# valida-xyz/valida

Measured on AMD Instinct MI355X. Metric: proofs/sec, 2^20-row Fibonacci trace, higher is better.
Workload: dtype u32; 1 GPU; C2: Fibonacci 2^20 cpu rows (mem 2^22), 14 chips, one proof per GPU; field=BabyBear / Ext5, mmcs=Keccak-256, fri_blowup=2, log_blowup=1, num_queries=40, pow_bits=8, parallelism=single GPU, proofs_in_flight_per_gpu=3, comm_stuck=False

## Files before the change

### bindings/rust/src/lib.rs

```rust
#![allow(non_camel_case_types, dead_code)]
use core::ffi::{c_char, c_int, c_void};

pub const VGPU_CBOR_CANONICAL_FIELDS: u32 = 1;
pub const VGPU_CBOR_PLAIN_DIGESTS: u32 = 2;
pub const VGPU_CBOR_IN_BARE_IS_MONTGOMERY: u32 = 1;
pub const VGPU_CBOR_SAW_FIELD_STRUCT: u32 = 1;
pub const VGPU_CBOR_SAW_FIELD_BARE: u32 = 2;
pub const VGPU_CBOR_SAW_DIGEST_STRUCT: u32 = 4;
pub const VGPU_CBOR_SAW_DIGEST_PLAIN: u32 = 8;
pub const VGPU_COMM_ID_BYTES: u32 = 128;
pub const VGPU_OK: i32 = 0;
pub const VGPU_ERR_INVALID_ARG: i32 = -1;
pub const VGPU_ERR_OOM: i32 = -2;
pub const VGPU_ERR_HIP: i32 = -3;
pub const VGPU_ERR_UNSUPPORTED: i32 = -4;
pub const VGPU_ERR_INTERNAL: i32 = -5;
pub const VGPU_ERR_FABRIC: i32 = -6;
pub const VGPU_HASH_KECCAK256: i32 = 0;
pub const VGPU_HASH_POSEIDON16: i32 = 1;
pub const VGPU_CPU_STORE32: i32 = 0;
pub const VGPU_CPU_LOAD32: i32 = 1;
pub const VGPU_CPU_JAL: i32 = 2;
pub const VGPU_CPU_JALV: i32 = 3;
pub const VGPU_CPU_BEQ: i32 = 4;
// ... 239 lines not shown
    pub mem_first: u32,
}
#[repr(C)]
#[derive(Clone, Copy)]
pub struct VgpuMemOp {
    pub clk: u32,
    pub addr: u32,
    pub value: u32,
    pub is_write: u32,
}
#[repr(C)]
#[derive(Clone, Copy)]
pub struct VgpuAluOp {
    pub opcode: u32,
    pub a: u32,
    pub b: u32,
    pub c: u32,
}
#[repr(C)]
#[derive(Clone, Copy)]
pub struct VgpuOutOp {
    pub clk: u32,
    pub byte: u32,
}
#[repr(C)]
#[derive(Clone, Copy)]
pub struct VgpuOplogDesc {
    pub struct_size: u64,
    pub cpu: *const VgpuCpuOp,
    pub n_cpu: u64,
    pub mem: *const VgpuMemOp,
    pub n_mem: u64,
    pub alu: [*const VgpuAluOp; 4],
    pub n_alu: [u64; 4],
    pub static_cells: *const u32,
    pub n_static: u64,
    pub rom_len: u32,
    pub alu2: [*const VgpuAluOp; 4],
    pub n_alu2: [u64; 4],
    pub output: *const VgpuOutOp,
    pub n_output: u64,
}

#[link(name = "vgpu")]
extern "C" {
    pub fn vgpu_last_error() -> *const c_char;
    pub fn vgpu_version() -> *const c_char;
    pub fn vgpu_air_new(name: *const c_char, width: u32, preprocessed_width: u32, out: *mut *mut VgpuAir) -> i32;
    pub fn vgpu_air_free(air: *mut VgpuAir);
    pub fn vgpu_air_constant(air: *mut VgpuAir, canonical: u32) -> u32;
    pub fn vgpu_air_variable(air: *mut VgpuAir, is_preprocessed: u32, column: u32, is_next: u32) -> u32;
    pub fn vgpu_air_is_first_row(air: *mut VgpuAir) -> u32;
    pub fn vgpu_air_is_last_row(air: *mut VgpuAir) -> u32;
    pub fn vgpu_air_is_transition(air: *mut VgpuAir) -> u32;
    pub fn vgpu_air_add(air: *mut VgpuAir, a: u32, b: u32) -> u32;
    pub fn vgpu_air_sub(air: *mut VgpuAir, a: u32, b: u32) -> u32;
    pub fn vgpu_air_mul(air: *mut VgpuAir, a: u32, b: u32) -> u32;
    pub fn vgpu_air_neg(air: *mut VgpuAir, a: u32) -> u32;
    pub fn vgpu_air_assert_zero(air: *mut VgpuAir, node: u32);
    pub fn vgpu_air_add_interaction(air: *mut VgpuAir, it: *const VgpuInteraction) -> i32;
    pub fn vgpu_machine_new(out: *mut *mut VgpuMachine) -> i32;
    pub fn vgpu_machine_push_air(m: *mut VgpuMachine, air: *const VgpuAir) -> i32;
    pub fn vgpu_machine_basic(out: *mut *mut VgpuMachine) -> i32;
    pub fn vgpu_machine_basic_via_ffi(out: *mut *mut VgpuMachine) -> i32;
    pub fn vgpu_machine_free(m: *mut VgpuMachine);
    pub fn vgpu_machine_num_chips(m: *const VgpuMachine) -> u32;
    pub fn vgpu_machine_chip_info(m: *const VgpuMachine, chip: u32, out: *mut u32) -> i32;
    pub fn vgpu_machine_interaction_words(m: *const VgpuMachine, chip: u32, out: *mut u32, cap: u64) -> i64;
    pub fn vgpu_machine_eval_constraints(m: *const VgpuMachine, chip: u32, main_local: *const u32, main_next: *const u32, prep_local: *const u32, prep_next: *const u32, is_first: u32, is_last: u32, is_transition: u32, out: *mut u32, cap: u32) -> i32;
    pub fn vgpu_challenger_new(poseidon_rc: *const u32, out: *mut *mut VgpuChallenger) -> i32;
    pub fn vgpu_challenger_free(ch: *mut VgpuChallenger);
    pub fn vgpu_challenger_observe(ch: *mut VgpuChallenger, values: *const u32, n: u64);
    pub fn vgpu_challenger_sample(ch: *mut VgpuChallenger, out: *mut u32, n: u64);
    pub fn vgpu_challenger_sample_bits(ch: *mut VgpuChallenger, bits: u32) -> u64;
    pub fn vgpu_challenger_grind(ch: *mut VgpuChallenger, bits: u32) -> u32;
    pub fn vgpu_poseidon16_permute(poseidon_rc: *const u32, state: *mut u32);
    pub fn vgpu_poseidon16_permute_sparse(poseidon_rc: *const u32, state: *mut u32) -> i32;
    pub fn vgpu_prover_create(cfg: *const VgpuConfig, machine: *const VgpuMachine, out: *mut *mut VgpuProver) -> i32;
    pub fn vgpu_prover_destroy(p: *mut VgpuProver);
    pub fn vgpu_prover_memory(p: *const VgpuProver, live_bytes: *mut u64, peak_bytes: *mut u64);
    pub fn vgpu_prover_trim(p: *mut VgpuProver) -> u64;
    pub fn vgpu_prover_memory_reset_peak(p: *mut VgpuProver);
    pub fn vgpu_prover_set_dense_lane(p: *mut VgpuProver, on: u32, min_nodes: u64);
    pub fn vgpu_prover_lane_stats(p: *const VgpuProver, entered: *mut u64, waited: *mut u64);
    pub fn vgpu_prover_set_profiling(p: *mut VgpuProver, on: u32);
    pub fn vgpu_prover_set_prep_cache(p: *mut VgpuProver, on: u32);
    pub fn vgpu_prover_set_profiling_filter(p: *mut VgpuProver, kernel_name: *const c_char);
    pub fn vgpu_prover_profile(p: *mut VgpuProver, out: *mut c_char, cap: u64) -> i64;
    pub fn vgpu_shader_clock_probe(device: i32, iters: u32, out: *mut u64) -> i32;
    pub fn vgpu_host_alloc(bytes: u64, out: *mut *mut c_void) -> i32;
    pub fn vgpu_host_free(ptr: *mut c_void);
    pub fn vgpu_trace_upload(p: *mut VgpuProver, data: *const u32, height: u64, width: u64, out: *mut *mut VgpuTrace) -> i32;
    pub fn vgpu_trace_free(t: *mut VgpuTrace);
    pub fn vgpu_commit_batches(p: *mut VgpuProver, mats: *const *const VgpuTrace, n_mats: u32, coset_shifts: *const u32, root: *mut u32, out: *mut *mut VgpuPdata) -> i32;
    pub fn vgpu_pdata_lde(p: *mut VgpuProver, pd: *const VgpuPdata, idx: u32, out: *mut u32, cap_words: u64) -> i32;
    pub fn vgpu_pdata_num_matrices(pd: *const VgpuPdata) -> u32;
    pub fn vgpu_pdata_lde_view(pd: *const VgpuPdata, idx: u32, out: *mut VgpuLdeView) -> i32;
    pub fn vgpu_pdata_free(pd: *mut VgpuPdata);
    pub fn vgpu_perm_trace(p: *mut VgpuProver, chip: u32, main: *const VgpuTrace, preprocessed_or_null: *const VgpuTrace, challenges: *const u32, out: *mut u32, cap_words: u64, cumulative_sum: *mut u32) -> i32;
    pub fn vgpu_perm_trace_device(p: *mut VgpuProver, chip: u32, main: *const VgpuTrace, preprocessed_or_null: *const VgpuTrace, challenges: *const u32, out: *mut *mut VgpuTrace, cumulative_sum: *mut u32) -> i32;
    pub fn vgpu_quotient(p: *mut VgpuProver, chip: u32, prep_pd: *const VgpuPdata, prep_idx: u32, main_pd: *const VgpuPdata, main_idx: u32, perm_pd: *const VgpuPdata, perm_idx: u32, perm_challenges: *const u32, alpha: *const u32, cumulative_sum: *const u32, out: *mut *mut VgpuTrace) -> i32;
    pub fn vgpu_open_multi_batches(p: *mut VgpuProver, rounds: *const *const VgpuPdata, n_rounds: u32, n_points: *const u32, points: *const u32, ch: *mut VgpuChallenger, out: *mut *mut VgpuOpening) -> i32;
    pub fn vgpu_opening_values_len(o: *const VgpuOpening) -> u64;
    pub fn vgpu_opening_values(o: *const VgpuOpening) -> *const u32;
    pub fn vgpu_opening_proof_len(o: *const VgpuOpening) -> u64;
    pub fn vgpu_opening_proof(o: *const VgpuOpening) -> *const u32;
    pub fn vgpu_opening_free(o: *mut VgpuOpening);
    pub fn vgpu_verify_multi_batches(cfg: *const VgpuConfig, commits: *const u32, n_rounds: u32, n_mats: *const u32, heights: *const u64, widths: *const u32, n_points: *const u32, points: *const u32, values: *const u32, n_value_words: u64, proof: *const u32, n_proof_words: u64, ch: *mut VgpuChallenger) -> i32;
    pub fn vgpu_verify(cfg: *const VgpuConfig, machine: *const VgpuMachine, preprocessed_commit: *const u32, proof_words: *const u32, n_words: u64) -> i32;
    pub fn vgpu_verifier_create(cfg: *const VgpuConfig, machine: *const VgpuMachine, out: *mut *mut VgpuVerifier) -> i32;
    pub fn vgpu_verifier_destroy(v: *mut VgpuVerifier);
    pub fn vgpu_verifier_set_chunk_words(v: *mut VgpuVerifier, chunk_words: u64) -> i32;
    pub fn vgpu_verify_batch(v: *mut VgpuVerifier, proofs: *const *const u32, n_words: *const u64, preprocessed_commits: *const u32, n_proofs: u32, status: *mut i32) -> i32;
    pub fn vgpu_verifier_message(v: *const VgpuVerifier, i: u32, out: *mut c_char, cap: u64) -> i64;
    pub fn vgpu_verifier_timing(v: *const VgpuVerifier, host_ms: *mut f64, device_ms: *mut f64);
    pub fn vgpu_host_commit_root(cfg: *const VgpuConfig, mats: *const *const u32, heights: *const u64, widths: *const u64, n_mats: u32, coset_shifts: *const u32, root: *mut u32) -> i32;
    pub fn vgpu_fri_fold(p: *mut VgpuProver, f: *const u32, n: u64, beta: *const u32, out: *mut u32) -> i32;
    pub fn vgpu_field_probe(p: *mut VgpuProver, op: u32, operands: *const u32, operand_words: u64, n_items: u64, results: *mut u32, result_words: u64) -> i32;
    pub fn vgpu_prover_set_pool_poison(p: *mut VgpuProver, mode: u32, word: u32) -> i32;
    pub fn vgpu_prover_pool_poison_stats(p: *const VgpuProver, out: *mut u64);
    pub fn vgpu_prover_pool_peek(p: *mut VgpuProver, bytes: u64, out: *mut u32, n_words: u64) -> i32;
    pub fn vgpu_verifier_set_poison(v: *mut VgpuVerifier, on: u32, word: u32) -> i32;
    pub fn vgpu_prove(p: *mut VgpuProver, main: *const *const VgpuTrace, n_main: u32, prep_chips: *const u32, prep: *const *const VgpuTrace, n_prep: u32, debug_flags: u32, out: *mut *mut VgpuProof) -> i32;
    pub fn vgpu_prove_async(p: *mut VgpuProver, main: *const *const VgpuTrace, n_main: u32, prep_chips: *const u32, prep: *const *const VgpuTrace, n_prep: u32, out: *mut *mut VgpuTicket) -> i32;
    pub fn vgpu_ticket_wait(t: *mut VgpuTicket, out: *mut *mut VgpuProof) -> i32;
    pub fn vgpu_proof_cbor(proof_words: *const u32, n_words: u64, flags: u32, out: *mut u8, cap_bytes: u64) -> i64;
    pub fn vgpu_proof_from_cbor(bytes: *const u8, n_bytes: u64, out: *mut u32, cap_words: u64) -> i64;
    pub fn vgpu_proof_from_cbor_ex(bytes: *const u8, n_bytes: u64, flags: u32, out: *mut u32, cap_words: u64, forms_seen: *mut u32) -> i64;
    pub fn vgpu_proof_len(pr: *const VgpuProof) -> u64;
    pub fn vgpu_proof_words(pr: *const VgpuProof) -> *const u32;
    pub fn vgpu_proof_phase_ms(pr: *const VgpuProof, out: *mut f64);
    pub fn vgpu_proof_transcript(pr: *const VgpuProof, out: *mut u32);
    pub fn vgpu_proof_debug_perm_trace(pr: *const VgpuProof, chip: u32, out: *mut u32, cap_words: u64) -> i64;
    pub fn vgpu_proof_debug_quotient(pr: *const VgpuProof, chip: u32, out: *mut u32, cap_words: u64) -> i64;
    pub fn vgpu_proof_free(pr: *mut VgpuProof);
    pub fn vgpu_bus_audit(p: *mut VgpuProver, main: *const *const VgpuTrace, n_main: u32, prep_chips: *const u32, prep: *const *const VgpuTrace, n_prep: u32, opts: *const VgpuBusAuditOpts, out: *mut *mut VgpuBusReport) -> i32;
    pub fn vgpu_bus_audit_host(machine: *const VgpuMachine, main: *const *const u32, heights: *const u64, widths: *const u64, n_main: u32, prep_chips: *const u32, prep: *const *const u32, prep_heights: *const u64, prep_widths: *const u64, n_prep: u32, opts: *const VgpuBusAuditOpts, out: *mut *mut VgpuBusReport) -> i32;
    pub fn vgpu_bus_report_len(r: *const VgpuBusReport) -> u64;
    pub fn vgpu_bus_report_words(r: *const VgpuBusReport) -> *const u32;
    pub fn vgpu_bus_report_timing(r: *const VgpuBusReport, out: *mut f64);
    pub fn vgpu_bus_report_free(r: *mut VgpuBusReport);
    pub fn vgpu_constraint_audit(p: *mut VgpuProver, main: *const *const VgpuTrace, n_main: u32, prep_chips: *const u32, prep: *const *const VgpuTrace, n_prep: u32, opts: *const VgpuConstraintAuditOpts, out: *mut *mut VgpuConstraintReport) -> i32;
    pub fn vgpu_constraint_audit_host(machine: *const VgpuMachine, main: *const *const u32, heights: *const u64, widths: *const u64, n_main: u32, prep_chips: *const u32, prep: *const *const u32, prep_heights: *const u64, prep_widths: *const u64, n_prep: u32, opts: *const VgpuConstraintAuditOpts, out: *mut *mut VgpuConstraintReport) -> i32;
    pub fn vgpu_constraint_report_len(r: *const VgpuConstraintReport) -> u64;
    pub fn vgpu_constraint_report_words(r: *const VgpuConstraintReport) -> *const u32;
    pub fn vgpu_constraint_report_timing(r: *const VgpuConstraintReport, out: *mut f64);
    pub fn vgpu_constraint_report_free(r: *mut VgpuConstraintReport);
    pub fn vgpu_mutation_audit(p: *mut VgpuProver, main: *const *const VgpuTrace, n_main: u32, prep_chips: *const u32, prep: *const *const VgpuTrace, n_prep: u32, opts: *const VgpuMutationAuditOpts, out: *mut *mut VgpuMutationReport) -> i32;
    pub fn vgpu_mutation_audit_host(machine: *const VgpuMachine, main: *const *const u32, heights: *const u64, widths: *const u64, n_main: u32, prep_chips: *const u32, prep: *const *const u32, prep_heights: *const u64, prep_widths: *const u64, n_prep: u32, opts: *const VgpuMutationAuditOpts, out: *mut *mut VgpuMutationReport) -> i32;
    pub fn vgpu_mutation_report_len(r: *const VgpuMutationReport) -> u64;
    pub fn vgpu_mutation_report_words(r: *const VgpuMutationReport) -> *const u32;
    pub fn vgpu_mutation_report_timing(r: *const VgpuMutationReport, out: *mut f64);
    pub fn vgpu_mutation_report_free(r: *mut VgpuMutationReport);
    pub fn vgpu_pair_audit(p: *mut VgpuProver, main: *const *const VgpuTrace, n_main: u32, prep_chips: *const u32, prep: *const *const VgpuTrace, n_prep: u32, opts: *const VgpuPairAuditOpts, out: *mut *mut VgpuPairReport) -> i32;
    pub fn vgpu_pair_audit_host(machine: *const VgpuMachine, main: *const *const u32, heights: *const u64, widths: *const u64, n_main: u32, prep_chips: *const u32, prep: *const *const u32, prep_heights: *const u64, prep_widths: *const u64, n_prep: u32, opts: *const VgpuPairAuditOpts, out: *mut *mut VgpuPairReport) -> i32;
    pub fn vgpu_pair_report_len(r: *const VgpuPairReport) -> u64;
    pub fn vgpu_pair_report_words(r: *const VgpuPairReport) -> *const u32;
    pub fn vgpu_pair_report_timing(r: *const VgpuPairReport, out: *mut f64);
    pub fn vgpu_pair_report_free(r: *mut VgpuPairReport);
    pub fn vgpu_rank_audit(p: *mut VgpuProver, main: *const *const VgpuTrace, n_main: u32, prep_chips: *const u32, prep: *const *const VgpuTrace, n_prep: u32, opts: *const VgpuRankAuditOpts, out: *mut *mut VgpuRankReport) -> i32;
    pub fn vgpu_rank_audit_host(machine: *const VgpuMachine, main: *const *const u32, heights: *const u64, widths: *const u64, n_main: u32, prep_chips: *const u32, prep: *const *const u32, prep_heights: *const u64, prep_widths: *const u64, n_prep: u32, opts: *const VgpuRankAuditOpts, out: *mut *mut VgpuRankReport) -> i32;
    pub fn vgpu_rank_report_len(r: *const VgpuRankReport) -> u64;
    pub fn vgpu_rank_report_words(r: *const VgpuRankReport) -> *const u32;
    pub fn vgpu_rank_report_timing(r: *const VgpuRankReport, out: *mut f64);
    pub fn vgpu_rank_report_free(r: *mut VgpuRankReport);
    pub fn vgpu_field_audit(p: *mut VgpuProver, main: *const *const VgpuTrace, n_main: u32, prep_chips: *const u32, prep: *const *const VgpuTrace, n_prep: u32, opts: *const VgpuRankAuditOpts, out: *mut *mut VgpuFieldReport) -> i32;
    pub fn vgpu_field_audit_host(machine: *const VgpuMachine, main: *const *const u32, heights: *const u64, widths: *const u64, n_main: u32, prep_chips: *const u32, prep: *const *const u32, prep_heights: *const u64, prep_widths: *const u64, n_prep: u32, opts: *const VgpuRankAuditOpts, out: *mut *mut VgpuFieldReport) -> i32;
    pub fn vgpu_field_report_len(r: *const VgpuFieldReport) -> u64;
    pub fn vgpu_field_report_words(r: *const VgpuFieldReport) -> *const u32;
    pub fn vgpu_field_report_timing(r: *const VgpuFieldReport, out: *mut f64);
    pub fn vgpu_field_report_free(r: *mut VgpuFieldReport);
    pub fn vgpu_link_audit(p: *mut VgpuProver, main: *const *const VgpuTrace, n_main: u32, prep_chips: *const u32, prep: *const *const VgpuTrace, n_prep: u32, opts: *const VgpuLinkAuditOpts, out: *mut *mut VgpuLinkReport) -> i32;
    pub fn vgpu_link_audit_host(machine: *const VgpuMachine, main: *const *const u32, heights: *const u64, widths: *const u64, n_main: u32, prep_chips: *const u32, prep: *const *const u32, prep_heights: *const u64, prep_widths: *const u64, n_prep: u32, opts: *const VgpuLinkAuditOpts, out: *mut *mut VgpuLinkReport) -> i32;
    pub fn vgpu_link_report_len(r: *const VgpuLinkReport) -> u64;
    pub fn vgpu_link_report_words(r: *const VgpuLinkReport) -> *const u32;
    pub fn vgpu_link_report_timing(r: *const VgpuLinkReport, out: *mut f64);
    pub fn vgpu_link_report_free(r: *mut VgpuLinkReport);
// ... 82 lines not shown
```

### include/vgpu.h

```cpp
#ifndef VGPU_H
#define VGPU_H
#include <stdint.h>
#ifdef __cplusplus
extern "C" {
#endif

enum {
    VGPU_OK = 0,
    VGPU_ERR_INVALID_ARG = -1,
    VGPU_ERR_OOM = -2,
    VGPU_ERR_HIP = -3,
    VGPU_ERR_UNSUPPORTED = -4,
    VGPU_ERR_INTERNAL = -5,
    VGPU_ERR_FABRIC = -6
};
enum {
    VGPU_HASH_KECCAK256 = 0,
    VGPU_HASH_POSEIDON16 = 1
};

const char* vgpu_last_error(void);
const char* vgpu_version(void);

typedef struct vgpu_config {
    int32_t device;
    uint32_t log_blowup;
    uint32_t num_queries;
    uint32_t pow_bits;
    uint32_t hash_kind;
    uint32_t observe_final_poly;
    uint32_t poseidon_rc[480];
    uint32_t interpret_air;
} vgpu_config_t;

typedef struct vgpu_air vgpu_air_t;
typedef struct vgpu_vcol_term { uint32_t is_preprocessed; uint32_t column; uint32_t weight; } vgpu_vcol_term_t;
typedef struct vgpu_vcol { const vgpu_vcol_term_t* terms; uint32_t n_terms; uint32_t constant; } vgpu_vcol_t;
typedef struct vgpu_interaction {
    const vgpu_vcol_t* fields; uint32_t n_fields;
    vgpu_vcol_t count;
    uint32_t is_global;
    uint32_t bus_index;
    uint32_t is_send;
} vgpu_interaction_t;

int32_t vgpu_air_new(const char* name, uint32_t width, uint32_t preprocessed_width, vgpu_air_t** out);
void vgpu_air_free(vgpu_air_t* air);
uint32_t vgpu_air_constant(vgpu_air_t* air, uint32_t canonical);
uint32_t vgpu_air_variable(vgpu_air_t* air, uint32_t is_preprocessed, uint32_t column, uint32_t is_next);
uint32_t vgpu_air_is_first_row(vgpu_air_t* air);
uint32_t vgpu_air_is_last_row(vgpu_air_t* air);
uint32_t vgpu_air_is_transition(vgpu_air_t* air);
uint32_t vgpu_air_add(vgpu_air_t* air, uint32_t a, uint32_t b);
uint32_t vgpu_air_sub(vgpu_air_t* air, uint32_t a, uint32_t b);
uint32_t vgpu_air_mul(vgpu_air_t* air, uint32_t a, uint32_t b);
uint32_t vgpu_air_neg(vgpu_air_t* air, uint32_t a);
void vgpu_air_assert_zero(vgpu_air_t* air, uint32_t node);
int32_t vgpu_air_add_interaction(vgpu_air_t* air, const vgpu_interaction_t* it);

typedef struct vgpu_machine vgpu_machine_t;
int32_t vgpu_machine_new(vgpu_machine_t** out);
int32_t vgpu_machine_push_air(vgpu_machine_t* m, const vgpu_air_t* air);
int32_t vgpu_machine_basic(vgpu_machine_t** out);
int32_t vgpu_machine_basic_via_ffi(vgpu_machine_t** out);
void vgpu_machine_free(vgpu_machine_t* m);
uint32_t vgpu_machine_num_chips(const vgpu_machine_t* m);
int32_t vgpu_machine_chip_info(const vgpu_machine_t* m, uint32_t chip, uint32_t out[8]);
int64_t vgpu_machine_interaction_words(const vgpu_machine_t* m, uint32_t chip, uint32_t* out, uint64_t cap);
int32_t vgpu_machine_eval_constraints(const vgpu_machine_t* m, uint32_t chip, const uint32_t* main_local, const uint32_t* main_next,
                                      const uint32_t* prep_local, const uint32_t* prep_next, uint32_t is_first, uint32_t is_last,
                                      uint32_t is_transition, uint32_t* out, uint32_t cap);

typedef struct vgpu_challenger vgpu_challenger_t;
int32_t vgpu_challenger_new(const uint32_t poseidon_rc[480], vgpu_challenger_t** out);
void vgpu_challenger_free(vgpu_challenger_t* ch);
void vgpu_challenger_observe(vgpu_challenger_t* ch, const uint32_t* values, uint64_t n);
void vgpu_challenger_sample(vgpu_challenger_t* ch, uint32_t* out, uint64_t n);
uint64_t vgpu_challenger_sample_bits(vgpu_challenger_t* ch, uint32_t bits);
uint32_t vgpu_challenger_grind(vgpu_challenger_t* ch, uint32_t bits);
void vgpu_poseidon16_permute(const uint32_t poseidon_rc[480], uint32_t state[16]);
int32_t vgpu_poseidon16_permute_sparse(const uint32_t poseidon_rc[480], uint32_t state[16]);

typedef struct vgpu_prover vgpu_prover_t;
typedef struct vgpu_trace vgpu_trace_t;
typedef struct vgpu_pdata vgpu_pdata_t;
typedef struct vgpu_proof vgpu_proof_t;

int32_t vgpu_prover_create(const vgpu_config_t* cfg, const vgpu_machine_t* machine, vgpu_prover_t** out);
void vgpu_prover_destroy(vgpu_prover_t* p);
void vgpu_prover_memory(const vgpu_prover_t* p, uint64_t* live_bytes, uint64_t* peak_bytes);
uint64_t vgpu_prover_trim(vgpu_prover_t* p);
void vgpu_prover_memory_reset_peak(vgpu_prover_t* p);
void vgpu_prover_set_dense_lane(vgpu_prover_t* p, uint32_t on, uint64_t min_nodes);
void vgpu_prover_lane_stats(const vgpu_prover_t* p, uint64_t* entered, uint64_t* waited);

void vgpu_prover_set_profiling(vgpu_prover_t* p, uint32_t on);
void vgpu_prover_set_prep_cache(vgpu_prover_t* p, uint32_t on);
void vgpu_prover_set_profiling_filter(vgpu_prover_t* p, const char* kernel_name);
int64_t vgpu_prover_profile(vgpu_prover_t* p, char* out, uint64_t cap);
int32_t vgpu_shader_clock_probe(int32_t device, uint32_t iters, uint64_t out[2]);

int32_t vgpu_host_alloc(uint64_t bytes, void** out);
void vgpu_host_free(void* ptr);

int32_t vgpu_trace_upload(vgpu_prover_t* p, const uint32_t* data, uint64_t height, uint64_t width, vgpu_trace_t** out);
void vgpu_trace_free(vgpu_trace_t* t);

int32_t vgpu_commit_batches(vgpu_prover_t* p, const vgpu_trace_t* const* mats, uint32_t n_mats, const uint32_t* coset_shifts,
                            uint32_t root[8], vgpu_pdata_t** out);
int32_t vgpu_pdata_lde(vgpu_prover_t* p, const vgpu_pdata_t* pd, uint32_t idx, uint32_t* out, uint64_t cap_words);
typedef struct vgpu_lde_view {
    const uint32_t* data;
    uint64_t height, width, stride;
    uint32_t log_blowup;
} vgpu_lde_view_t;
uint32_t vgpu_pdata_num_matrices(const vgpu_pdata_t* pd);
int32_t vgpu_pdata_lde_view(const vgpu_pdata_t* pd, uint32_t idx, vgpu_lde_view_t* out);
void vgpu_pdata_free(vgpu_pdata_t* pd);

int32_t vgpu_perm_trace(vgpu_prover_t* p, uint32_t chip, const vgpu_trace_t* main, const vgpu_trace_t* preprocessed_or_null,
                        const uint32_t challenges[15], uint32_t* out, uint64_t cap_words, uint32_t cumulative_sum[5]);

int32_t vgpu_perm_trace_device(vgpu_prover_t* p, uint32_t chip, const vgpu_trace_t* main, const vgpu_trace_t* preprocessed_or_null,
                               const uint32_t challenges[15], vgpu_trace_t** out, uint32_t cumulative_sum[5]);

int32_t vgpu_quotient(vgpu_prover_t* p, uint32_t chip, const vgpu_pdata_t* prep_pd, uint32_t prep_idx, const vgpu_pdata_t* main_pd, uint32_t main_idx,
                      const vgpu_pdata_t* perm_pd, uint32_t perm_idx, const uint32_t perm_challenges[15], const uint32_t alpha[5],
                      const uint32_t cumulative_sum[5], vgpu_trace_t** out);

typedef struct vgpu_opening vgpu_opening_t;
int32_t vgpu_open_multi_batches(vgpu_prover_t* p, const vgpu_pdata_t* const* rounds, uint32_t n_rounds, const uint32_t* n_points,
                                const uint32_t* points, vgpu_challenger_t* ch, vgpu_opening_t** out);
uint64_t vgpu_opening_values_len(const vgpu_opening_t* o);
const uint32_t* vgpu_opening_values(const vgpu_opening_t* o);
uint64_t vgpu_opening_proof_len(const vgpu_opening_t* o);
const uint32_t* vgpu_opening_proof(const vgpu_opening_t* o);
void vgpu_opening_free(vgpu_opening_t* o);

int32_t vgpu_verify_multi_batches(const vgpu_config_t* cfg, const uint32_t* commits, uint32_t n_rounds, const uint32_t* n_mats, const uint64_t* heights,
                                  const uint32_t* widths, const uint32_t* n_points, const uint32_t* points, const uint32_t* values, uint64_t n_value_words,
                                  const uint32_t* proof, uint64_t n_proof_words, vgpu_challenger_t* ch);

int32_t vgpu_verify(const vgpu_config_t* cfg, const vgpu_machine_t* machine, const uint32_t* preprocessed_commit, const uint32_t* proof_words,
                    uint64_t n_words);
typedef struct vgpu_verifier vgpu_verifier_t;
int32_t vgpu_verifier_create(const vgpu_config_t* cfg, const vgpu_machine_t* machine, vgpu_verifier_t** out);
void vgpu_verifier_destroy(vgpu_verifier_t* v);
int32_t vgpu_verifier_set_chunk_words(vgpu_verifier_t* v, uint64_t chunk_words);
int32_t vgpu_verify_batch(vgpu_verifier_t* v, const uint32_t* const* proofs, const uint64_t* n_words, const uint32_t* preprocessed_commits,
                          uint32_t n_proofs, int32_t* status);
int64_t vgpu_verifier_message(const vgpu_verifier_t* v, uint32_t i, char* out, uint64_t cap);
void vgpu_verifier_timing(const vgpu_verifier_t* v, double* host_ms, double* device_ms);
int32_t vgpu_host_commit_root(const vgpu_config_t* cfg, const uint32_t* const* mats, const uint64_t* heights, const uint64_t* widths, uint32_t n_mats,
                              const uint32_t* coset_shifts, uint32_t root[8]);

int32_t vgpu_fri_fold(vgpu_prover_t* p, const uint32_t* f, uint64_t n, const uint32_t beta[5], uint32_t* out);

int32_t vgpu_field_probe(vgpu_prover_t* p, uint32_t op, const uint32_t* operands, uint64_t operand_words, uint64_t n_items, uint32_t* results, uint64_t result_words);

int32_t vgpu_prover_set_pool_poison(vgpu_prover_t* p, uint32_t mode, uint32_t word);
void vgpu_prover_pool_poison_stats(const vgpu_prover_t* p, uint64_t out[4]);
int32_t vgpu_prover_pool_peek(vgpu_prover_t* p, uint64_t bytes, uint32_t* out, uint64_t n_words);
int32_t vgpu_verifier_set_poison(vgpu_verifier_t* v, uint32_t on, uint32_t word);

int32_t vgpu_prove(vgpu_prover_t* p, const vgpu_trace_t* const* main, uint32_t n_main, const uint32_t* prep_chips,
                   const vgpu_trace_t* const* prep, uint32_t n_prep, uint32_t debug_flags, vgpu_proof_t** out);
typedef struct vgpu_ticket vgpu_ticket_t;
int32_t vgpu_prove_async(vgpu_prover_t* p, const vgpu_trace_t* const* main, uint32_t n_main, const uint32_t* prep_chips,
                         const vgpu_trace_t* const* prep, uint32_t n_prep, vgpu_ticket_t** out);
int32_t vgpu_ticket_wait(vgpu_ticket_t* t, vgpu_proof_t** out);
#define VGPU_CBOR_CANONICAL_FIELDS 1u
#define VGPU_CBOR_PLAIN_DIGESTS 2u
int64_t vgpu_proof_cbor(const uint32_t* proof_words, uint64_t n_words, uint32_t flags, uint8_t* out, uint64_t cap_bytes);
int64_t vgpu_proof_from_cbor(const uint8_t* bytes, uint64_t n_bytes, uint32_t* out, uint64_t cap_words);
#define VGPU_CBOR_IN_BARE_IS_MONTGOMERY 1u
#define VGPU_CBOR_SAW_FIELD_STRUCT 1u
#define VGPU_CBOR_SAW_FIELD_BARE 2u
#define VGPU_CBOR_SAW_DIGEST_STRUCT 4u
#define VGPU_CBOR_SAW_DIGEST_PLAIN 8u
int64_t vgpu_proof_from_cbor_ex(const uint8_t* bytes, uint64_t n_bytes, uint32_t flags, uint32_t* out, uint64_t cap_words, uint32_t* forms_seen);
uint64_t vgpu_proof_len(const vgpu_proof_t* pr);
const uint32_t* vgpu_proof_words(const vgpu_proof_t* pr);
void vgpu_proof_phase_ms(const vgpu_proof_t* pr, double out[11]);
void vgpu_proof_transcript(const vgpu_proof_t* pr, uint32_t out[33]);
int64_t vgpu_proof_debug_perm_trace(const vgpu_proof_t* pr, uint32_t chip, uint32_t* out, uint64_t cap_words);
int64_t vgpu_proof_debug_quotient(const vgpu_proof_t* pr, uint32_t chip, uint32_t* out, uint64_t cap_words);
void vgpu_proof_free(vgpu_proof_t* pr);

typedef struct vgpu_bus_audit_opts { uint64_t max_tuples; uint32_t max_records_per_tuple; uint32_t hash_bits; } vgpu_bus_audit_opts_t;
typedef struct vgpu_bus_report vgpu_bus_report_t;
int32_t vgpu_bus_audit(vgpu_prover_t* p, const vgpu_trace_t* const* main, uint32_t n_main, const uint32_t* prep_chips, const vgpu_trace_t* const* prep,
                       uint32_t n_prep, const vgpu_bus_audit_opts_t* opts, vgpu_bus_report_t** out);
// ... 339 lines not shown
```

### valida_amd/__init__.py

```python
import ctypes
import os

import numpy as np

P = 2013265921
NUM_CHIPS = 14
CHIP_NAMES = ["cpu", "program", "mem", "add", "sub", "mul", "div", "shift", "lt", "com", "bitwise", "output", "range", "static_data"]

_HERE = os.path.dirname(os.path.abspath(__file__))
_LIB_PATH = os.environ.get("VGPU_LIB_PATH") or os.path.join(_HERE, "libvgpu.so")

c_u32p = ctypes.POINTER(ctypes.c_uint32)
c_u64p = ctypes.POINTER(ctypes.c_uint64)


HASH_KECCAK256, HASH_POSEIDON16 = 0, 1


class VgpuError(RuntimeError):
    def __init__(self, code, msg):
        super().__init__("vgpu error %d: %s" % (code, msg))
        self.code = code


# ... 1973 lines not shown
        return cls(cls._image(first.deltas, False, len(listed), chips, listed))


def _coverage_opts(deltas, max_cells, max_workgroups):
    if int(max_cells) < 1:
        raise VgpuError(-1, "coverage_audit: max_cells must be at least 1")
    ds = [int(d) for d in ((1, P - 1) if deltas is None else deltas)]
    if not 1 <= len(ds) <= 4:
        raise VgpuError(-1, "coverage_audit: 1 to 4 deltas (got %d)" % len(ds))
    if any(d < 0 or d > 0xFFFFFFFF for d in ds):
        raise VgpuError(-1, "coverage_audit: a delta must be a canonical value in 1..p-1")
    if not 0 <= int(max_workgroups) <= 0xFFFFFFFF:
        raise VgpuError(-1, "coverage_audit: max_workgroups is a 32-bit count (0: the default)")
    return CoverageAuditOpts(int(max_cells), len(ds), (ctypes.c_uint32 * 4)(*ds), int(max_workgroups), (ctypes.c_uint32 * 2)(0, 0))


def coverage_audit_host(machine, main_matrices, preprocessed, deltas=None, max_cells=8192):
    opts = _coverage_opts(deltas, max_cells, 0)
    return _audit_host("coverage", machine, main_matrices, preprocessed, opts)


_AUDIT_REPORTS = dict(bus=BusReport, constraint=ConstraintReport, mutation=MutationReport, pair=PairReport, rank=RankReport, step=StepReport, invariant=InvariantReport, transition=TransitionReport, product=ProductReport, domain=DomainReport, memory=MemoryReport, program=ProgramReport, field=FieldReport,
                      link=LinkReport, coverage=CoverageReport)


def _report_of(name):
    return lambda h: _audit_report(name, _AUDIT_REPORTS[name], h)


_rank_report, _step_report, _field_report, _link_report = _report_of("rank"), _report_of("step"), _report_of("field"), _report_of("link")

def _pool_poison_from_env(environ):
    text = environ.get("VGPU_POOL_POISON", "").strip()
    if not text:
        return None
    hexa = text[:2] in ("0x", "0X")
    digits = text[2:] if hexa else text
    if not digits or any(ch not in ("0123456789abcdefABCDEF" if hexa else "0123456789") for ch in digits):
        raise ValueError("VGPU_POOL_POISON must be a 32-bit word in decimal or 0x hex, not %r" % text)
    word = int(digits, 16 if hexa else 10)
    if word > 0xFFFFFFFF:
        raise ValueError("VGPU_POOL_POISON must be a 32-bit word (at most 0xFFFFFFFF), not %r" % text)
    return word


class Ticket:

    def __init__(self, handle, keep):
        self._h, self._keep = handle, keep

    def wait(self):
        h = ctypes.c_void_p()
        t, self._h = self._h, None
        _check(lib().vgpu_ticket_wait(t, ctypes.byref(h)))
        self._keep = None
        return Proof(h)

    def __del__(self):
        if getattr(self, "_h", None):
            try:
                self.wait()
            except Exception:
                pass


class Prover:

    def __init__(self, machine, rc, device=0, log_blowup=1, num_queries=40, pow_bits=8, observe_final_poly=False, interpret_air=False, hash_kind=HASH_KECCAK256):
        cfg = VgpuConfig()
        cfg.device, cfg.log_blowup, cfg.num_queries, cfg.pow_bits = device, log_blowup, num_queries, pow_bits
        cfg.hash_kind, cfg.observe_final_poly, cfg.interpret_air = int(hash_kind), int(observe_final_poly), int(interpret_air)
        rc = np.ascontiguousarray(rc, dtype=np.uint32)
        assert rc.size == 480
        ctypes.memmove(cfg.poseidon_rc, rc.ctypes.data, 480 * 4)
        self.machine, self.rc, self.log_blowup, self.num_queries, self.pow_bits = machine, rc, log_blowup, num_queries, pow_bits
        self._h = ctypes.c_void_p()
        lane_off, lane_min = os.environ.get("VGPU_DENSE_LANE", "1") == "0", os.environ.get("VGPU_DENSE_LANE_MIN_NODES", "").strip()
        if lane_min and not lane_min.isdigit():
            raise ValueError("VGPU_DENSE_LANE_MIN_NODES must be a number of leaf rows, not %r" % lane_min)
        poison = _pool_poison_from_env(os.environ)
        _check(lib().vgpu_prover_create(ctypes.byref(cfg), machine._h, ctypes.byref(self._h)))
        if lane_off or int(lane_min or 0) > 0:
            self.set_dense_lane(not lane_off, int(lane_min or 0))
        if poison is not None:
            self.set_pool_poison(poison)

    def set_dense_lane(self, on, min_nodes=0):
        lib().vgpu_prover_set_dense_lane(self._h, ctypes.c_uint32(1 if on else 0), ctypes.c_uint64(int(min_nodes)))

    def upload(self, matrix):
        m = np.ascontiguousarray(matrix, dtype=np.uint32)
        assert m.ndim == 2
        h = ctypes.c_void_p()
        _check(lib().vgpu_trace_upload(self._h, m.ctypes.data_as(c_u32p), ctypes.c_uint64(m.shape[0]), ctypes.c_uint64(m.shape[1]), ctypes.byref(h)))
        return DeviceTrace(self, h, m.shape)

    def upload_oplog(self, desc):
        h = ctypes.c_void_p()
        _check(lib().vgpu_oplog_upload(self._h, ctypes.byref(desc), ctypes.byref(h)))
        nbytes = 48 * desc.n_cpu + 16 * desc.n_mem + 16 * sum(desc.n_alu) + 8 * desc.n_static
        log = DeviceOplog(self, h, int(nbytes))
        log._desc = desc
        return log

    def generate_trace(self, log, chip):
        h = ctypes.c_void_p()
        _check(lib().vgpu_generate_trace(self._h, log._h, ctypes.c_uint32(chip), ctypes.byref(h)))
        hh, ww = ctypes.c_uint64(), ctypes.c_uint64()
        lib().vgpu_trace_shape(h, ctypes.byref(hh), ctypes.byref(ww))
        return DeviceTrace(self, h, (int(hh.value), int(ww.value)))

    def commit_batches(self, traces, coset_shifts=None):
        arr = (ctypes.c_void_p * len(traces))(*[t._h for t in traces])
        root = np.zeros(8, dtype=np.uint32)
        sh = None
        if coset_shifts is not None:
            shv, sh = _u32(coset_shifts)
        h = ctypes.c_void_p()
        _check(lib().vgpu_commit_batches(self._h, arr, ctypes.c_uint32(len(traces)), sh, root.ctypes.data_as(c_u32p), ctypes.byref(h)))
        return ProverData(self, h, root, [t.shape for t in traces])

    def generate_permutation_trace(self, chip, main, challenges, preprocessed=None):
        info = self.machine.chip_info(chip)
        n = main.shape[0]
        out = np.zeros((n, 5 * (info["interactions"] + 1)), dtype=np.uint32)
        ch, chp = _u32(challenges)
        cs = np.zeros(5, dtype=np.uint32)
        _check(lib().vgpu_perm_trace(self._h, ctypes.c_uint32(chip), main._h, preprocessed._h if preprocessed is not None else None, chp,
                                     out.ctypes.data_as(c_u32p), ctypes.c_uint64(out.size), cs.ctypes.data_as(c_u32p)))
        return out, cs

    def permutation_trace_device(self, chip, main, challenges, preprocessed=None):
        ch, chp = _u32(challenges)
        cs = np.zeros(5, dtype=np.uint32)
        h = ctypes.c_void_p()
        _check(lib().vgpu_perm_trace_device(self._h, ctypes.c_uint32(chip), main._h, preprocessed._h if preprocessed is not None else None, chp, ctypes.byref(h),
                                            cs.ctypes.data_as(c_u32p)))
        hh, ww = ctypes.c_uint64(), ctypes.c_uint64()
        lib().vgpu_trace_shape(h, ctypes.byref(hh), ctypes.byref(ww))
        return DeviceTrace(self, h, (int(hh.value), int(ww.value))), cs

    def quotient(self, chip, main_pd, main_idx, perm_pd, perm_idx, perm_challenges, alpha, cumulative_sum, prep_pd=None, prep_idx=0):
        a, ap = _u32(perm_challenges)
        b, bp = _u32(alpha)
        c, cp = _u32(cumulative_sum)
        h = ctypes.c_void_p()
        _check(lib().vgpu_quotient(self._h, ctypes.c_uint32(chip), prep_pd._h if prep_pd is not None else None, ctypes.c_uint32(prep_idx), main_pd._h,
                                   ctypes.c_uint32(main_idx), perm_pd._h, ctypes.c_uint32(perm_idx), ap, bp, cp, ctypes.byref(h)))
        hh, ww = ctypes.c_uint64(), ctypes.c_uint64()
        lib().vgpu_trace_shape(h, ctypes.byref(hh), ctypes.byref(ww))
        return DeviceTrace(self, h, (int(hh.value), int(ww.value)))

    def open_multi_batches(self, rounds, points, challenger):
        arr = (ctypes.c_void_p * len(rounds))(*[r._h for r in rounds])
        n_points = np.array([len(pts) for rnd in points for pts in rnd], dtype=np.uint32)
        flat = np.array([w for rnd in points for pts in rnd for z in pts for w in z], dtype=np.uint32)
        h = ctypes.c_void_p()
        _check(lib().vgpu_open_multi_batches(self._h, arr, ctypes.c_uint32(len(rounds)), n_points.ctypes.data_as(c_u32p), flat.ctypes.data_as(c_u32p), challenger._h,
                                             ctypes.byref(h)))
        L = lib()
        for f in (L.vgpu_opening_values_len, L.vgpu_opening_proof_len):
            f.restype = ctypes.c_uint64
        for f in (L.vgpu_opening_values, L.vgpu_opening_proof):
            f.restype = c_u32p
        try:
            nv, npf = int(L.vgpu_opening_values_len(h)), int(L.vgpu_opening_proof_len(h))
            vals = np.ctypeslib.as_array(L.vgpu_opening_values(h), shape=(nv,)).copy() if nv else np.zeros(0, np.uint32)
            proof = np.ctypeslib.as_array(L.vgpu_opening_proof(h), shape=(npf,)).copy()
        finally:
            L.vgpu_opening_free(h)
        out, pos = [], 0
        for r, rnd in enumerate(points):
            out.append([])
            for i, pts in enumerate(rnd):
                w = rounds[r]._shapes[i][1]
                out[r].append([])
                for _ in pts:
                    out[r][i].append(vals[pos:pos + 5 * w].reshape(w, 5))
                    pos += 5 * w
        assert pos == vals.size
        return out, proof

    def fri_fold(self, f, beta):
        f = np.ascontiguousarray(f, dtype=np.uint32)
        n = f.shape[0]
        b, bp = _u32(beta)
        out = np.zeros((n // 2, 5), dtype=np.uint32)
        _check(lib().vgpu_fri_fold(self._h, f.ctypes.data_as(c_u32p), ctypes.c_uint64(n), bp, out.ctypes.data_as(c_u32p)))
        return out

    def prove(self, main, preprocessed, debug=False, check=False):
        arr = (ctypes.c_void_p * len(main))(*[t._h for t in main])
        chips = (ctypes.c_uint32 * max(1, len(preprocessed)))(*[c for c, _ in preprocessed])
        parr = (ctypes.c_void_p * max(1, len(preprocessed)))(*[t._h for _, t in preprocessed])
        h = ctypes.c_void_p()
        _check(lib().vgpu_prove(self._h, arr, ctypes.c_uint32(len(main)), chips, parr, ctypes.c_uint32(len(preprocessed)),
                                ctypes.c_uint32((1 if debug else 0) | (2 if check else 0)), ctypes.byref(h)))
        return Proof(h)

    def _audit(self, name, main, preprocessed, opts):
        arr = (ctypes.c_void_p * max(1, len(main)))(*[t._h for t in main])
        chips = (ctypes.c_uint32 * max(1, len(preprocessed)))(*[c for c, _ in preprocessed])
        parr = (ctypes.c_void_p * max(1, len(preprocessed)))(*[t._h for _, t in preprocessed])
# ... 126 lines not shown
```

### valida_amd/csrc/capi.cpp

```cpp
#include "../../include/vgpu.h"
#include <algorithm>
#include <cstring>
#include <future>
#include <map>
#include <mutex>
#include <memory>
#include <string>
#include "host/cbor.hpp"
#include "host/comm.hpp"
#include "host/sharded.hpp"
#include "host/sharded_prover.hpp"
#include "host/verifier.hpp"
#include "host/machine_verifier.hpp"
#include "host/verify_batch.hpp"
#include "host/poseidon_opt.hpp"
#include "host/prover.hpp"
#include "workload/basic_vm.hpp"
#include "workload/executable.hpp"

using namespace vhost;

static thread_local std::string g_err;
static int32_t fail(int32_t code, const std::string& msg) { g_err = msg; return code; }
#define VG_TRY(...)                                                         \
// ... 231 lines not shown
    };
    const auto& its = m->desc.airs[chip].interactions;
    w.push_back((uint32_t)its.size());
    for (auto& it : its) {
        w.push_back(it.is_send() ? 1u : 0u); w.push_back(it.is_local() ? 0u : 1u); w.push_back((uint32_t)it.bus_index); w.push_back((uint32_t)it.fields.size());
        vcol(it.count);
        for (auto& f : it.fields) vcol(f);
    }
    if (out && cap >= w.size()) memcpy(out, w.data(), w.size() * 4);
    return (int64_t)w.size();
}
int32_t vgpu_machine_eval_constraints(const vgpu_machine_t* m, uint32_t chip, const uint32_t* main_local, const uint32_t* main_next,
                                      const uint32_t* prep_local, const uint32_t* prep_next, uint32_t is_first, uint32_t is_last,
                                      uint32_t is_transition, uint32_t* out, uint32_t cap) {
    try {
        if (!m || chip >= m->desc.airs.size()) throw std::invalid_argument("bad chip index");
        const AirDesc& a = m->desc.airs[chip];
        std::vector<Fp> ml(a.width), mn(a.width), pl(a.prep_width), pn(a.prep_width);
        for (uint32_t i = 0; i < a.width; i++) { ml[i] = Fp::from_canonical(main_local[i]); mn[i] = Fp::from_canonical(main_next[i]); }
        for (uint32_t i = 0; i < a.prep_width; i++) { pl[i] = Fp::from_canonical(prep_local[i]); pn[i] = Fp::from_canonical(prep_next[i]); }
        vair::HostEval ev{ml.data(), mn.data(), pl.data(), pn.data(), Fp::from_canonical(is_first), Fp::from_canonical(is_last), Fp::from_canonical(is_transition)};
        auto vals = ev.run(a.program);
        if (vals.size() > cap) throw std::invalid_argument("output buffer too small");
        for (size_t i = 0; i < vals.size(); i++) out[i] = vals[i].canonical();
        return (int32_t)vals.size();
    } catch (const std::exception& e) { return fail(VGPU_ERR_INVALID_ARG, e.what()); }
}

int32_t vgpu_challenger_new(const uint32_t rc[480], vgpu_challenger_t** out) {
    VG_TRY({
        if (!rc || !out) throw std::invalid_argument("null argument");
        auto* c = new vgpu_challenger();
        c->perm.reset(new Poseidon16(rc));
        c->ch.reset(new Challenger(c->perm.get()));
        *out = c;
    })
}
void vgpu_challenger_free(vgpu_challenger_t* ch) { delete ch; }
void vgpu_challenger_observe(vgpu_challenger_t* ch, const uint32_t* v, uint64_t n) { for (uint64_t i = 0; i < n; i++) ch->ch->observe_canonical(v[i]); }
void vgpu_challenger_sample(vgpu_challenger_t* ch, uint32_t* out, uint64_t n) { for (uint64_t i = 0; i < n; i++) out[i] = ch->ch->sample().canonical(); }
uint64_t vgpu_challenger_sample_bits(vgpu_challenger_t* ch, uint32_t bits) { return ch->ch->sample_bits(bits); }
uint32_t vgpu_challenger_grind(vgpu_challenger_t* ch, uint32_t bits) { return ch->ch->grind(bits); }
void vgpu_poseidon16_permute(const uint32_t rc[480], uint32_t state[16]) {
    Poseidon16 p(rc);
    Fp st[16];
    for (int i = 0; i < 16; i++) st[i] = Fp::from_canonical(state[i]);
    p.permute(st);
    for (int i = 0; i < 16; i++) state[i] = st[i].canonical();
}

int32_t vgpu_poseidon16_permute_sparse(const uint32_t rc[480], uint32_t state[16]) {
    Poseidon16 p(rc);
    PoseidonOptTables t(p);
    if (!t.valid) return VGPU_ERR_UNSUPPORTED;
    Fp st[16];
    for (int i = 0; i < 16; i++) st[i] = Fp::from_canonical(state[i]);
    t.permute(p, st);
    for (int i = 0; i < 16; i++) state[i] = st[i].canonical();
    return VGPU_OK;
}

int32_t vgpu_prover_create(const vgpu_config_t* cfg, const vgpu_machine_t* machine, vgpu_prover_t** out) {
    VG_TRY({
        if (!cfg || !machine || !out) throw std::invalid_argument("null argument");
        if (cfg->hash_kind != VGPU_HASH_KECCAK256 && cfg->hash_kind != VGPU_HASH_POSEIDON16) { g_err = "hash_kind must be VGPU_HASH_KECCAK256 or VGPU_HASH_POSEIDON16"; return VGPU_ERR_UNSUPPORTED; }
        if (cfg->log_blowup < 1 || cfg->log_blowup > 4) throw std::invalid_argument("log_blowup must be in 1..4");
        int count = 0;
        if (hipGetDeviceCount(&count) != hipSuccess || count <= cfg->device) throw std::runtime_error("hip: no usable device (the product path has no CPU fallback)");
        FriParams fp;
        fp.log_blowup = cfg->log_blowup; fp.num_queries = cfg->num_queries; fp.pow_bits = cfg->pow_bits; fp.observe_final_poly = cfg->observe_final_poly != 0;
        fp.interpret_air = cfg->interpret_air != 0;
        fp.hash_kind = (int)cfg->hash_kind;
        auto* p = new vgpu_prover();
        p->p.reset(new Prover(cfg->device, machine->desc, cfg->poseidon_rc, fp));
        *out = p;
    })
}
void vgpu_prover_destroy(vgpu_prover_t* p) { delete p; }
void vgpu_prover_memory(const vgpu_prover_t* p, uint64_t* live, uint64_t* peak) {
    auto& c = const_cast<vgpu_prover_t*>(p)->p->ctx();
    if (live) *live = c.live;
    if (peak) *peak = c.peak_live;
}
void vgpu_prover_set_dense_lane(vgpu_prover_t* p, uint32_t on, uint64_t min_nodes) {
    if (!p) return;
    DeviceCtx& c = p->p->ctx();
    std::lock_guard<std::mutex> lk(c.prove_mu);
    c.lane_on = on != 0;
    if (min_nodes) c.lane_min_nodes = min_nodes;
}
void vgpu_prover_lane_stats(const vgpu_prover_t* p, uint64_t* entered, uint64_t* waited) {
    if (!p) return;
    auto& c = const_cast<vgpu_prover_t*>(p)->p->ctx();
    if (entered) *entered = c.lane_entered.load();
    if (waited) *waited = c.lane_waited.load();
}
void vgpu_prover_memory_reset_peak(vgpu_prover_t* p) {
    if (!p) return;
    DeviceCtx& c = p->p->ctx();
    std::lock_guard<std::mutex> lk(c.pool_mu);
    c.peak_live = c.live;
}
uint64_t vgpu_prover_trim(vgpu_prover_t* p) {
    if (!p) return 0;
    DeviceCtx& c = p->p->ctx();
    (void)hipSetDevice(c.device);
    return (uint64_t)c.trim();
}
void vgpu_prover_set_profiling(vgpu_prover_t* p, uint32_t on) {
    auto& c = p->p->ctx();
    c.profiler.reset();
    c.profiler.enabled = on != 0;
}
int32_t vgpu_shader_clock_probe(int32_t device, uint32_t iters, uint64_t out[2]) {
    VG_TRY({
        if (!out || !iters) throw std::invalid_argument("shader_clock_probe: null output or zero iterations");
        struct Probe { hipStream_t st = nullptr; uint64_t* buf = nullptr; };
        static std::mutex mu;
        static std::map<int, Probe> probes;
        std::lock_guard<std::mutex> lk(mu);
        VG_HIP_CHECK(hipSetDevice(device));
        Probe& pr = probes[device];
        if (!pr.st) {
            VG_HIP_CHECK(hipStreamCreateWithFlags(&pr.st, hipStreamNonBlocking));
            VG_HIP_CHECK(hipHostMalloc((void**)&pr.buf, 64));
        }
        pr.buf[0] = pr.buf[1] = 0;
        vk::launch_clock_probe(pr.st, pr.buf, iters);
        VG_HIP_CHECK(hipStreamSynchronize(pr.st));
        if (!pr.buf[1]) throw std::runtime_error("hip: the clock probe wrote nothing");
        out[0] = pr.buf[0]; out[1] = pr.buf[1];
    })
}
void vgpu_prover_set_prep_cache(vgpu_prover_t* p, uint32_t on) { if (p) p->p->set_prep_cache(on != 0); }
void vgpu_prover_set_profiling_filter(vgpu_prover_t* p, const char* kernel_name) { p->p->ctx().profiler.only = kernel_name ? kernel_name : ""; }
int64_t vgpu_prover_profile(vgpu_prover_t* p, char* out, uint64_t cap) {
    std::string s;
    {
        DeviceCtx& c = p->p->ctx();
        (void)hipSetDevice(c.device);
        (void)hipDeviceSynchronize();
        c.profiler.collect();
    }
    for (auto& kv : p->p->ctx().profiler.stats) {
        char line[256];
        snprintf(line, sizeof line, "%s %llu %.6f %.0f %.0f\n", kv.first.c_str(), (unsigned long long)kv.second.launches, kv.second.ms, kv.second.bytes,
                 kv.second.valu_ops);
        s += line;
    }
    if (out && cap > s.size()) memcpy(out, s.c_str(), s.size() + 1);
    return (int64_t)s.size() + 1;
}
int32_t vgpu_host_alloc(uint64_t bytes, void** out) {
    VG_TRY({
        if (!out || !bytes) throw std::invalid_argument("vgpu_host_alloc: null output or zero size");
        void* ptr = nullptr;
        hipError_t e = hipHostMalloc(&ptr, bytes, hipHostMallocPortable);
        if (e == hipErrorOutOfMemory) throw std::bad_alloc();
        if (e != hipSuccess) throw std::runtime_error(std::string("hipHostMalloc: ") + hipGetErrorString(e));
        *out = ptr;
    })
}
void vgpu_host_free(void* ptr) { if (ptr) (void)hipHostFree(ptr); }
int32_t vgpu_trace_upload(vgpu_prover_t* p, const uint32_t* data, uint64_t height, uint64_t width, vgpu_trace_t** out) {
    VG_TRY({
        if (!p || !data || !out || !height || !width) throw std::invalid_argument("bad trace");
// ... 36 lines not shown
                if (!good) throw std::invalid_argument(std::string("oplog: ") + chip + " log entry " + std::to_string(i) + " has an opcode that is not an operation of that chip");
                if (k == 2 && h.alu2[k][i].c >= 32) throw std::invalid_argument("oplog: shift log entry " + std::to_string(i) + ": shift amount >= 32");
            }
        };
        check(0, {OP_MUL32, OP_MULHS32, OP_MULHU32}, "mul");
        check(1, {OP_DIV32, OP_SDIV32}, "div");
        check(2, {OP_SHL32, OP_SHR32, OP_SRA32}, "shift");
        check(3, {OP_NE32, OP_EQ32}, "com");
    }
    for (uint64_t i = 1; i < h.n_static; i++)
        if (log->static_cells[2 * i] <= log->static_cells[2 * i - 2]) throw std::invalid_argument("oplog: static cells must be in ascending address order");
    if (!h.n_cpu || !log->cpu) throw std::invalid_argument("oplog: empty cpu log");
    if ((h.n_mem && !log->mem) || (h.n_static && !log->static_cells)) throw std::invalid_argument("oplog: null log with a nonzero length");
    for (int k = 0; k < 4; k++) if (h.n_alu[k] && !h.alu[k]) throw std::invalid_argument("oplog: null ALU log with a nonzero length");
    for (uint64_t i = 0; i < h.n_cpu; i++) {
        const vgpu_cpu_op_t& o = log->cpu[i];
        if (o.mem_first > h.n_mem || (i && o.mem_first < log->cpu[i - 1].mem_first) || o.kind > VGPU_CPU_READ_ADVICE)
            throw std::invalid_argument("oplog: cpu record " + std::to_string(i) + " is malformed");
        if (h.rom_len && o.pc >= h.rom_len) throw std::invalid_argument("oplog: cpu record " + std::to_string(i) + ": pc beyond the ROM length");
        if (o.kind == VGPU_CPU_BUS || o.kind == VGPU_CPU_BUS_LEFT_IMM) {
            using namespace vchips;
            const uint32_t op = o.opcode;
            const bool known = (op >= OP_ADD32 && op <= OP_SLE32) || op == OP_WRITE;
            if (!known) throw std::invalid_argument("oplog: cpu record " + std::to_string(i) + ": opcode " + std::to_string(op) + " is no bus operation of the BasicMachine's chips");
        }
    }
    for (uint64_t i = 1; i < h.n_mem; i++)
        if (log->mem[i].clk < log->mem[i - 1].clk) throw std::invalid_argument("oplog: memory log entry " + std::to_string(i) + " is out of clock order");
    return h;
}
int32_t vgpu_oplog_validate(const vgpu_oplog_desc_t* log) {
    VG_TRY({
        if (!log) throw std::invalid_argument("null argument");
        checked_oplog(log);
    })
}
int32_t vgpu_oplog_upload(vgpu_prover_t* p, const vgpu_oplog_desc_t* log, vgpu_oplog_t** out) {
    VG_TRY({
        if (!p || !log || !out) throw std::invalid_argument("null argument");
        const HostOplog h = checked_oplog(log);
        p->p->ctx().activate();
        std::unique_ptr<vgpu_oplog> l(new vgpu_oplog());
        l->owner = p->p;
        l->log = p->p->upload_oplog(h);
        *out = l.release();
    })
}
void vgpu_oplog_free(vgpu_oplog_t* log) { delete log; }
int32_t vgpu_generate_trace(vgpu_prover_t* p, const vgpu_oplog_t* log, uint32_t chip, vgpu_trace_t** out) {
    VG_TRY({
        if (!p || !log || !out) throw std::invalid_argument("null argument");
        p->p->ctx().activate();
        std::unique_ptr<vgpu_trace> t(new vgpu_trace());
        t->owner = p->p;
        t->t = p->p->generate_trace(*log->log, (int)chip);
        *out = t.release();
    })
}

static DMat ingest(DeviceCtx& c, const DeviceTrace& t) {
    if (t.height & (t.height - 1)) throw std::invalid_argument("matrix height must be a power of two");
    DMat m(&c, t.height, t.width);
    if (!t.nat.empty()) VG_HIP_CHECK(hipMemcpyAsync(m.data, t.nat.data, t.height * t.width * 4, hipMemcpyDeviceToDevice, c.stream));
    else vk::launch_ingest(c.stream, t.raw.data, m.view(), false);
    return m;
}

int32_t vgpu_commit_batches(vgpu_prover_t* p, const vgpu_trace_t* const* mats, uint32_t n_mats, const uint32_t* coset_shifts, uint32_t root[8],
                            vgpu_pdata_t** out) {
    VG_TRY({
        if (!p || !mats || !n_mats || !root || !out) throw std::invalid_argument("null argument");
        DeviceCtx& c = p->p->ctx();
        c.activate();
        std::vector<DMat> nat;
        for (uint32_t i = 0; i < n_mats; i++) { if (!mats[i] || mats[i]->owner != p->p) throw std::invalid_argument("null trace or trace of another prover"); nat.push_back(ingest(c, *mats[i]->t)); }
        std::vector<CommitInput> in;
        for (uint32_t i = 0; i < n_mats; i++) in.push_back({&nat[i], mats[i]->t->nat_rows_bitrev, mats[i]->t->nat_rows_bitrev});
        std::vector<Fp> shifts;
        if (coset_shifts) for (uint32_t i = 0; i < n_mats; i++) shifts.push_back(Fp::from_canonical(coset_shifts[i]));
        std::unique_ptr<vgpu_pdata> pd(new vgpu_pdata());
        pd->owner = p->p;
        pd->pd = commit_batches(&c, in, coset_shifts ? &shifts : nullptr, p->p->fri());
        memcpy(root, pd->pd->tree.root, 32);
        *out = pd.release();
    })
}
int32_t vgpu_pdata_lde(vgpu_prover_t* p, const vgpu_pdata_t* pd, uint32_t idx, uint32_t* out, uint64_t cap_words) {
    VG_TRY({
        if (!p || !pd || idx >= pd->pd->ldes.size() || !out) throw std::invalid_argument("bad argument");
        DeviceCtx& c = p->p->ctx();
        c.activate();
        const DMat& l = pd->pd->ldes[idx];
        if (cap_words < l.height * l.width) throw std::invalid_argument("output buffer too small");
        DBuf tmp(&c, (size_t)(l.height * l.width));
        vk::launch_export_rows(c.stream, l.view(), 0, l.height, tmp.data);
        c.download(out, tmp.data, l.height * l.width * 4);
    })
}
uint32_t vgpu_pdata_num_matrices(const vgpu_pdata_t* pd) { return pd ? (uint32_t)pd->pd->ldes.size() : 0; }
int32_t vgpu_pdata_lde_view(const vgpu_pdata_t* pd, uint32_t idx, vgpu_lde_view_t* out) {
    VG_TRY({
        if (!pd || !out || idx >= pd->pd->ldes.size()) throw std::invalid_argument("bad argument");
        const DMat& l = pd->pd->ldes[idx];
        out->data = l.data; out->height = l.height; out->width = l.width; out->stride = l.height;
        out->log_blowup = pd->owner->fri().log_blowup;
    })
}
void vgpu_pdata_free(vgpu_pdata_t* pd) { delete pd; }

static Ext5 ext_of(const uint32_t* w) { Ext5 e; for (int k = 0; k < 5; k++) e.c[k] = Fp::from_canonical(w[k]); return e; }

int32_t vgpu_perm_trace_device(vgpu_prover_t* p, uint32_t chip, const vgpu_trace_t* main, const vgpu_trace_t* prep, const uint32_t challenges[15],
                               vgpu_trace_t** out, uint32_t cumulative_sum[5]) {
    VG_TRY({
        if (!p || !main || !challenges || !out) throw std::invalid_argument("null argument");
        const MachineDesc& md = p->p->machine();
        if (chip >= md.airs.size()) throw std::invalid_argument("bad chip index");
        if (main->t->width != md.airs[chip].width) throw std::invalid_argument("trace width mismatch");
        DeviceCtx& c = p->p->ctx();
        c.activate();
        DMat m = ingest(c, *main->t);
        DMat pm;
        if (prep) pm = ingest(c, *prep->t);
        Ext5 rnd[3] = {ext_of(challenges), ext_of(challenges + 5), ext_of(challenges + 10)};
        Ext5 cs;
        std::unique_ptr<vgpu_trace> t(new vgpu_trace());
        t->owner = p->p;
        t->t = std::make_shared<DeviceTrace>();
        t->t->nat = p->p->permutation_trace((int)chip, m, prep ? &pm : nullptr, rnd, &cs);
        t->t->height = t->t->nat.height; t->t->width = t->t->nat.width;
        if (cumulative_sum) for (int k = 0; k < 5; k++) cumulative_sum[k] = cs.c[k].canonical();
        *out = t.release();
    })
}

int32_t vgpu_quotient(vgpu_prover_t* p, uint32_t chip, const vgpu_pdata_t* prep_pd, uint32_t prep_idx, const vgpu_pdata_t* main_pd, uint32_t main_idx,
                      const vgpu_pdata_t* perm_pd, uint32_t perm_idx, const uint32_t perm_challenges[15], const uint32_t alpha[5],
                      const uint32_t cumulative_sum[5], vgpu_trace_t** out) {
    VG_TRY({
        if (!p || !main_pd || !perm_pd || !perm_challenges || !alpha || !cumulative_sum || !out) throw std::invalid_argument("null argument");
        if (chip >= p->p->machine().airs.size()) throw std::invalid_argument("bad chip index");
        if (main_pd->owner != p->p || perm_pd->owner != p->p || (prep_pd && prep_pd->owner != p->p)) throw std::invalid_argument("prover data of another prover context");
        if (main_idx >= main_pd->pd->ldes.size() || perm_idx >= perm_pd->pd->ldes.size() || (prep_pd && prep_idx >= prep_pd->pd->ldes.size()))
            throw std::invalid_argument("bad matrix index");
        p->p->ctx().activate();
        Ext5 rnd[3] = {ext_of(perm_challenges), ext_of(perm_challenges + 5), ext_of(perm_challenges + 10)};
        std::unique_ptr<vgpu_trace> t(new vgpu_trace());
        t->owner = p->p;
        t->t = std::make_shared<DeviceTrace>();
        t->t->nat = p->p->quotient_chunks((int)chip, main_pd->pd->ldes[main_idx], perm_pd->pd->ldes[perm_idx], prep_pd ? &prep_pd->pd->ldes[prep_idx] : nullptr, rnd,
                                          ext_of(alpha), ext_of(cumulative_sum));
        t->t->nat_rows_bitrev = true;
        t->t->height = t->t->nat.height; t->t->width = t->t->nat.width;
        *out = t.release();
    })
}

int32_t vgpu_open_multi_batches(vgpu_prover_t* p, const vgpu_pdata_t* const* rounds, uint32_t n_rounds, const uint32_t* n_points, const uint32_t* points,
                                vgpu_challenger_t* ch, vgpu_opening_t** out) {
    VG_TRY({
        if (!p || !rounds || !n_rounds || !n_points || !points || !ch || !out) throw std::invalid_argument("null argument");
        std::vector<OpenRound> rs(n_rounds);
        size_t k = 0, w = 0;
        for (uint32_t r = 0; r < n_rounds; r++) {
            if (!rounds[r] || rounds[r]->owner != p->p) throw std::invalid_argument("null prover data or prover data of another prover context");
            rs[r].pd = rounds[r]->pd.get();
// ... 1193 lines not shown
```

### valida_amd/csrc/host/pcs.hpp

```cpp
#pragma once
#include <algorithm>
#include <functional>
#include <memory>
#include "fri_params.hpp"
#include "runtime.hpp"

namespace vhost {


struct ColMat {
    uint64_t height = 0;
    std::vector<const uint32_t*> cols;
};

struct DeviceTree {
    static constexpr uint64_t TOP_FIRST_LEN = 256;
    DeviceCtx* ctx = nullptr;
    std::vector<DBuf> layers;
    std::vector<uint64_t> layer_len;
    unsigned log_max_height = 0;
    uint32_t root[8] = {0};
    static constexpr uint64_t DROP_MIN_LEAVES = 1ull << 16;
    bool drop_bottom = false;
    unsigned dropped = 0;
// ... 84 lines not shown
            vk::launch_poseidon_levels(st, tab, c->poseidon_sparse, pgrp);
            pgrp.levels = 0;
        };
        auto add_level = [&](vk::KeccakTopArgs& g, uint64_t len, const Group* inj) {
            if (g.levels == 0) { g.prev = layers[layers.size() - 2].data; g.first_len = len; }
            g.out[g.levels] = layers.back().data;
            g.cols[g.levels] = inj ? pd + inj->first : nullptr;
            g.n_elems[g.levels] = inj ? (int)inj->count : 0;
            g.levels++;
        };
        auto flush_mid = [&] {
            if (!mid.levels) return;
            mid.block_len = vk::KECCAK_LEVELS_BLOCK_LEN;
            if (leaves_in_mid) {
                if (mid.prev != layers[0].data) throw std::logic_error("mmcs: leaf prologue without a launch over the leaf layer");
                mid.leaf_base = single_view->data; mid.leaf_stride = single_view->stride; mid.leaf_elems = (int)single_view->width; mid.leaf_rows = maxh;
            }
            vk::launch_keccak_levels(st, mid);
            mid.levels = 0;
        };
        for (uint64_t len = maxh / 2; len >= 1; len /= 2) {
            layers.emplace_back(c, (size_t)len * 8);
            layer_len.push_back(len);
            const Group* inj = (gi < groups.size() && groups[gi].height == len) ? &groups[gi] : nullptr;
            if (inj && before_injection_) { (*before_injection_)(); before_injection_ = nullptr; }
            if (pos ? vk::poseidon_levels_take(len) : (len <= TOP_FIRST_LEN || vk::keccak_levels_fused(len))) lane_guard.leave();
            if (pos) {
                if (!vk::poseidon_levels_take(len)) vk::launch_poseidon_compress(st, tab, c->poseidon_sparse, layers[layers.size() - 2].data, inj ? pd + inj->first : nullptr, inj ? (int)inj->count : 0, len, layers.back().data);
                else {
                    if (pgrp.levels && vk::poseidon_levels_group(len) != pgroup) flush_pos(false);
                    pgroup = vk::poseidon_levels_group(len);
                    add_level(pgrp, len, inj);
                }
            } else if (len > TOP_FIRST_LEN) {
                if (vk::keccak_levels_fused(len)) add_level(mid, len, inj);
                else vk::launch_keccak_compress(st, layers[layers.size() - 2].data, inj ? pd + inj->first : nullptr, inj ? (int)inj->count : 0, len,
                                                layers.back().data);
            } else {
                flush_mid();
                add_level(top, len, inj);
            }
            if (inj) gi++;
            if (len == 1) break;
        }
        lane_guard.leave();
        flush_mid();
        if (leaves_in_mid && layers.size() < 2) throw std::logic_error("mmcs: leaf prologue on a tree without parents");
        if (leaves_in_top) {
            if (!top.levels || top.prev != layers[0].data) throw std::logic_error("mmcs: leaf prologue without a top launch over the leaf layer");
            top.leaf_base = single_view->data; top.leaf_stride = single_view->stride; top.leaf_elems = (int)single_view->width; top.leaf_rows = maxh;
        }
        flush_pos(true);
        if (challenger_ && !pos) {
            if (!top.levels) throw std::logic_error("mmcs: the challenger epilogue needs a tree with at least one parent layer");
            top.ch_pos = challenger_->pos; top.ch_state = challenger_->state; top.ch_beta5 = challenger_->beta5; top.ch_commit8 = challenger_->commit8;
        }
        if (top.levels) vk::launch_keccak_top(st, top);
        if (gi != groups.size()) throw std::runtime_error("mmcs: matrix heights must be powers of two >= 1 and <= max height");
        c->check_launch("mmcs build");
        dropped = 0;
        if (drop_bottom && st == c->stream && !c->in_section && maxh >= DROP_MIN_LEAVES && layers.size() >= 4) {
            leaf_elems = (int)groups[0].count;
            if (single) { leaf_ptr = single_view->data; leaf_stride = single_view->stride; }
            else { leaf_ptr = pd + groups[0].first; leaf_stride = 0; }
            layers[0] = DBuf();
            dropped = 1;
            if (!(groups.size() > 1 && groups[1].height == maxh / 2)) { layers[1] = DBuf(); dropped = 2; }
        }
        if (fetch_root) c->download_small(root, layers.back().data, 32);
        if (!fetch_root || dropped) ptr_table_ = std::move(ptr_buf);
    }

};

struct ProverData {
    std::vector<DMat> ldes;
    DeviceTree tree;
};

struct CommitInput {
    DMat* mat;
    bool rows_bitrev;
    bool consume;
};

inline DMat coset_lde(DeviceCtx* c, hipStream_t st, const CommitInput& in, unsigned log_blowup, Fp lde_shift) {
    const uint64_t n = in.mat->height, b = 1ull << log_blowup;
    if (n == 0 || (n & (n - 1))) throw std::invalid_argument("commit: matrix heights must be powers of two");
    if (vg::log2_strict_u64(n) + log_blowup > 27)
        throw std::invalid_argument("commit: LDE height 2^" + std::to_string(vg::log2_strict_u64(n) + log_blowup) + " exceeds the field's two-adicity (2^27)");
    const unsigned k = vg::log2_strict_u64(n);
    static const bool fused = [] { const char* e = getenv("VGPU_LDE_FUSED"); return !(e && e[0] == '0'); }();
    if (!in.rows_bitrev && fused) {
        DMat lde(c, n * b, in.mat->width);
        const vk::LdeTables lt = c->lde_tables((int)k, (int)log_blowup, lde_shift);
        DMat s1, s2;
        if (k > 12) { s1 = DMat(c, n, in.mat->width); s2 = DMat(c, n * b, in.mat->width); }
        vk::launch_lde_natural(st, in.mat->view(), lde.view(), (int)log_blowup, c->tables, lt, s1.empty() ? vk::DMatView{nullptr, 0, 0, 0} : s1.view(),
                               s2.empty() ? vk::DMatView{nullptr, 0, 0, 0} : s2.view());
        c->check_launch("coset_lde");
        return lde;
    }
    DMat coeffs;
    if (in.rows_bitrev && in.consume) coeffs = std::move(*in.mat);
    else {
        coeffs = DMat(c, n, in.mat->width);
        if (in.rows_bitrev) VG_HIP_CHECK(hipMemcpyAsync(coeffs.data, in.mat->data, n * in.mat->width * 4, hipMemcpyDeviceToDevice, st));
        else vk::launch_bitrev_rows(st, in.mat->view(), coeffs.view());
    }
    vk::launch_intt(st, coeffs.view(), c->tables);
    DMat lde(c, n * b, coeffs.width);
    Fp w = vg::two_adic_generator(k + log_blowup), wt = Fp::one();
    for (uint64_t t = 0; t < b; t++) {
        uint64_t block = vg::reverse_bits_len((uint32_t)t, log_blowup);
        vk::launch_coset_ntt(st, coeffs.view(), lde.view(), block * n, lde_shift * wt, c->tables);
        wt *= w;
    }
    c->check_launch("coset_lde");
    return lde;
}

struct CommitRider {
    const std::vector<CommitInput>* mats;
    std::unique_ptr<ProverData>* out;
};
inline std::unique_ptr<ProverData> commit_batches(DeviceCtx* c, const std::vector<CommitInput>& mats, const std::vector<Fp>* coset_shifts,
                                                  const FriParams& fri, const CommitRider* rider = nullptr) {
    auto pd = std::make_unique<ProverData>();
    Fp g = Fp::from_canonical(vg::GENERATOR);
    uint64_t maxh = 0;
    for (auto& m : mats) maxh = std::max<uint64_t>(maxh, m.mat->height);
    Section lde_section(c);
    if (rider) {
        auto rp = std::make_unique<ProverData>();
        hipStream_t ax = c->aux[0];
        for (auto& m : *rider->mats) rp->ldes.push_back(coset_lde(c, ax, m, fri.log_blowup, g));
        std::vector<vk::DMatView> rviews;
        for (auto& l : rp->ldes) rviews.push_back(l.view());
        rp->tree.build(c, rviews, false, nullptr, nullptr, ax);
        VG_HIP_CHECK(hipMemcpyAsync(c->rider_root_pin, rp->tree.layers.back().data, 32, hipMemcpyDeviceToHost, ax));
        *rider->out = std::move(rp);
    }
    pd->ldes.resize(mats.size());
    for (int pass = 0; pass < 2; pass++)
        for (size_t i = 0; i < mats.size(); i++) {
            const bool tallest = mats[i].mat->height == maxh;
            if (tallest != (pass == 0)) continue;
            Fp shift = coset_shifts ? g * (*coset_shifts)[i].inv() : g;
            hipStream_t st = c->stream_for(i, mats[i].mat->height);
            pd->ldes[i] = coset_lde(c, st, mats[i], fri.log_blowup, shift);
        }
    std::vector<vk::DMatView> views;
    for (auto& l : pd->ldes) views.push_back(l.view());
    lde_section.join();
    pd->tree.drop_bottom = true;
    pd->tree.build(c, views);
    if (rider) {
        VG_HIP_CHECK(hipStreamSynchronize(c->aux[0]));
        memcpy((*rider->out)->tree.root, c->rider_root_pin, 32);
    }
    return pd;
}

}
```

### valida_amd/csrc/host/prover.cpp

```cpp
#include "prover.hpp"
#include "poseidon_opt.hpp"

namespace vhost {

static Ext5 ext_from_canonical(const uint32_t* w) { Ext5 e; for (int k = 0; k < 5; k++) e.c[k] = Fp::from_canonical(w[k]); return e; }
static void ext_to_canonical(const Ext5& e, uint32_t* w) { for (int k = 0; k < 5; k++) w[k] = e.c[k].canonical(); }

Prover::Prover(int device, const MachineDesc& machine, const uint32_t* poseidon_rc480, const FriParams& fri)
    : ctx_(new DeviceCtx(device)), machine_(machine), fri_(fri), perm16_(poseidon_rc480) {
    for (auto& a : machine_.airs) {
        if (a.log_quotient_degree < 1 || a.log_quotient_degree > 3) throw std::invalid_argument("chip " + a.name + ": log_quotient_degree must be 1..3");
        if (a.native_chip != -2 && (a.native_chip < 0 || a.native_chip >= 14)) throw std::invalid_argument("chip " + a.name + ": native_chip must be a BasicMachine chip id (0..13) or -2 (captured AIR)");
        if (a.log_quotient_degree != 1 && a.native_chip >= 0) throw std::invalid_argument("chip " + a.name + ": the compiled chip kernels assume log_quotient_degree = 1");
        if (fri_.log_blowup < a.log_quotient_degree)
            throw std::invalid_argument("chip " + a.name + ": log_blowup must be >= log_quotient_degree (the quotient domain must lie inside the committed LDE)");
        std::vector<uint32_t> pw(a.program.instrs.size() * 2 + 2, 0);
        if (!a.program.instrs.empty()) memcpy(pw.data(), a.program.instrs.data(), a.program.instrs.size() * 8);
        prog_dev_.emplace_back(ctx_.get(), pw);
        iw_dev_.emplace_back(ctx_.get(), a.interaction_words);
    }
    bool sparse = false;
    const std::vector<uint32_t> pos = poseidon_device_image(poseidon_rc480, perm16_, sparse);
    pow_pos_ = DBuf(ctx_.get(), pos);
    VG_HIP_CHECK(hipHostMalloc((void**)&cs_pinned_, CS_PINNED_WORDS * 4));
// ... 205 lines not shown
    vk::launch_perm_trace(c.stream, main_nat.view(), prep_nat ? prep_nat->view() : vk::DMatView{nullptr, 0, 0, 0}, iw_dev_[chip].data, pool_dev.data, M, perm.view(), scratch.data, fri_.interpret_air ? -2 : machine_.airs[(size_t)chip].native_chip);
    c.check_launch("perm trace");
    if (cumulative_sum) {
        GatherList gl;
        const uint64_t n = main_nat.height;
        gl.add(perm.data + (uint64_t)(5 * M) * n + (n - 1), n, 5, 0);
        DBuf gd(&c, gl.desc), gout(&c, 8);
        vk::launch_gather(c.stream, gd.data, gl.n(), gout.data);
        uint32_t cs[5];
        c.download(cs, gout.data, 20);
        *cumulative_sum = ext_from_canonical(cs);
    } else c.sync();
    return perm;
}

DMat Prover::quotient_chunks(int chip, const DMat& main_lde, const DMat& perm_lde, const DMat* prep_lde, const Ext5 rnd[3], const Ext5& alpha,
                             const Ext5& cumulative_sum) {
    DeviceCtx& c = *ctx_;
    const AirDesc& air = machine_.airs.at((size_t)chip);
    const unsigned lb = fri_.log_blowup;
    const unsigned log_n = vg::log2_strict_u64(main_lde.height) - lb;
    if (main_lde.width != air.width || perm_lde.width != 5 * (air.interactions.size() + 1) || perm_lde.height != main_lde.height ||
        (air.prep_width && (!prep_lde || prep_lde->width != air.prep_width || prep_lde->height != main_lde.height)))
        throw std::invalid_argument("quotient: LDE shapes do not match chip " + air.name);
    std::vector<uint32_t> pool;
    vk::QuotientArgs a{};
    a.K = quotient_consts(air, rnd, alpha, cumulative_sum, pool);
    DBuf pool_dev(&c, pool);
    fill_quotient_args(a, chip, main_lde.view(), perm_lde.view(), prep_lde ? prep_lde->view() : vk::DMatView{nullptr, 0, 0, 0}, log_n, pool_dev.data);
    DMat q(&c, 1ull << log_n, 5ull << air.log_quotient_degree);
    a.out = q.view();
    vk::launch_quotient(c.stream, a, c.tables);
    c.check_launch("quotient");
    c.sync();
    return q;
}

void Prover::fill_quotient_args(vk::QuotientArgs& a, int chip, vk::DMatView main_lde, vk::DMatView perm_lde, vk::DMatView prep_lde, unsigned log_n, const uint32_t* consts_dev) {
    const AirDesc& air = machine_.airs[(size_t)chip];
    const Fp s = Fp::from_canonical(vg::GENERATOR);
    a.main_lde = main_lde; a.perm_lde = perm_lde; a.prep_lde = prep_lde;
    a.log_n = (int)log_n;
    a.prog = (const vair::Instr*)prog_dev_[chip].data;
    a.n_instrs = (uint32_t)air.program.instrs.size();
    a.n_regs = air.program.num_regs;
    a.n_air_asserts = air.program.num_asserts;
    a.native_chip = fri_.interpret_air ? vk::QuotientArgs::INTERPRET : air.native_chip;
    a.iw = iw_dev_[chip].data;
    a.consts = consts_dev;
    a.coset_shift = s.v;
    a.coset_shift_inv = s.inv().v;
    a.lqd = (int)air.log_quotient_degree;
    const Fp sn = s.exp_power_of_2(log_n), wq = vg::two_adic_generator(air.log_quotient_degree);
    Fp wp = Fp::one();
    for (unsigned r = 0; r < (1u << air.log_quotient_degree); r++) { Fp z = sn * wp - Fp::one(); a.zh[r] = z.v; a.zh_inv[r] = z.inv().v; wp *= wq; }
    a.g_inv = vg::two_adic_generator(log_n).inv().v;
}


std::vector<uint32_t> Prover::prove(const std::vector<const DeviceTrace*>& main, const std::vector<std::pair<int, const DeviceTrace*>>& preprocessed,
                                    PhaseTimes* times, ProveDebugOut* dbg) {
    DeviceCtx& c = *ctx_;
    c.activate();
    std::unique_lock<std::mutex> one_at_a_time(c.prove_mu);
    c.activate();
    struct Running {
        std::atomic<int>& n;
        explicit Running(std::atomic<int>& a) : n(a) { n.fetch_add(1); }
        ~Running() { n.fetch_sub(1); }
    } running(c.proofs_running);
    struct LaneOpen { explicit LaneOpen(const DeviceCtx* x) { DeviceCtx::lane_thread_ctx() = x; } ~LaneOpen() { DeviceCtx::lane_thread_ctx() = nullptr; } } lane_open(&c);
    const size_t NC = machine_.airs.size();
    if (main.size() != NC) throw std::invalid_argument("prove: need one main trace per chip");
    const Fp s = Fp::from_canonical(vg::GENERATOR);
    const unsigned lb = fri_.log_blowup;
    Challenger ch(&perm16_);
    PhaseTimes tm;
    auto t_total = Clock::now();
    auto t0 = Clock::now();

    std::vector<unsigned> log_deg(NC);
    std::vector<DMat> main_own(NC);
    std::vector<const DMat*> main_nat(NC);
    Section ingest_section(&c);
    for (size_t i = 0; i < NC; i++) {
        if (main[i]->width != machine_.airs[i].width) throw std::invalid_argument("prove: trace width mismatch for chip " + machine_.airs[i].name);
        uint64_t h = main[i]->height;
        if (h == 0 || (h & (h - 1))) throw std::invalid_argument("prove: trace heights must be powers of two");
        log_deg[i] = vg::log2_strict_u64(h);
        if (!main[i]->nat.empty()) { main_nat[i] = &main[i]->nat; continue; }
        main_own[i] = DMat(&c, h, main[i]->width);
        main_nat[i] = &main_own[i];
        vk::launch_ingest(c.stream_for(i, h), main[i]->raw.data, main_own[i].view(), false);
    }
    std::vector<std::pair<int, uint64_t>> prep_key;
    for (auto& pr : preprocessed) prep_key.emplace_back(pr.first, pr.second->uid);
    const bool prep_hit = prep_cache_enabled_ && !prep_key.empty() && prep_key == prep_key_ && prep_pd_cache_;
    if (!prep_hit) { prep_key_.clear(); prep_pd_cache_.reset(); prep_nat_cache_.clear(); prep_nat_cache_.resize(preprocessed.size()); }
    std::vector<DMat>& prep_nat = prep_nat_cache_;
    struct DropPrep { Prover* p; ~DropPrep() { if (!p->prep_cache_enabled_) { p->prep_key_.clear(); p->prep_pd_cache_.reset(); p->prep_nat_cache_.clear(); } } } drop_prep{this};
    std::vector<int> prep_slot(NC, -1);
    for (size_t k = 0; k < preprocessed.size(); k++) {
        const DeviceTrace* t = preprocessed[k].second;
        int chip = preprocessed[k].first;
        if (chip < 0 || (size_t)chip >= NC || prep_slot[chip] >= 0) throw std::invalid_argument("prove: bad or repeated preprocessed chip index");
        if (t->width != machine_.airs[chip].prep_width || t->height != main[chip]->height) throw std::invalid_argument("prove: preprocessed trace shape mismatch");
        prep_slot[chip] = (int)k;
        if (prep_hit) continue;
        prep_nat[k] = DMat(&c, t->height, t->width);
        if (!t->nat.empty())
            VG_HIP_CHECK(hipMemcpyAsync(prep_nat[k].data, t->nat.data, t->height * t->width * 4, hipMemcpyDeviceToDevice, c.stream_for(k, t->height)));
        else
            vk::launch_ingest(c.stream_for(k, t->height), t->raw.data, prep_nat[k].view(), false);
    }
    ingest_section.join();
    c.check_launch("ingest");
    tm.ingest = ms_since(t0);

    t0 = Clock::now();
    ProverData* prep_pd = nullptr;
    std::vector<CommitInput> prep_in;
    const bool ride = !prep_nat.empty() && !prep_hit;
    if (ride)
        for (auto& m : prep_nat) prep_in.push_back({&m, false, false});
    std::unique_ptr<ProverData> main_pd;
    {
        std::vector<CommitInput> in;
        for (auto m : main_nat) in.push_back({const_cast<DMat*>(m), false, false});
        const CommitRider rider{&prep_in, &prep_pd_cache_};
        main_pd = commit_batches(&c, in, nullptr, fri_, ride ? &rider : nullptr);
    }
    if (!prep_nat.empty()) {
        if (!prep_hit && prep_cache_enabled_) prep_key_ = prep_key;
        prep_pd = prep_pd_cache_.get();
        ch.observe_digest(prep_pd->tree.root);
    }
    ch.observe_digest(main_pd->tree.root);
    tm.commit_main = ms_since(t0);

    t0 = Clock::now();
    Ext5 rnd[3];
    for (int i = 0; i < 3; i++) rnd[i] = ch.sample_ext();
    std::vector<std::vector<Ext5>> bus_alphas(NC), betas(NC);
    std::vector<DMat> perm_nat(NC);
    std::vector<Ext5> cumulative_sums(NC);
    uint32_t* cs_host = nullptr;
    DBuf cs_keep;
    {
        std::vector<uint32_t> pool;
        std::vector<size_t> off(NC);
        for (size_t i = 0; i < NC; i++) {
            auto& its = machine_.airs[i].interactions;
            size_t maxf = 0;
            for (auto& it : its) {
                const Ext5& r = it.is_local() ? rnd[0] : rnd[1];
                bus_alphas[i].push_back(r.pow((uint64_t)it.bus_index + 1));
                maxf = std::max(maxf, it.fields.size());
            }
            Ext5 bp = Ext5::one();
            for (size_t j = 0; j < maxf; j++) { betas[i].push_back(bp); bp *= rnd[2]; }
            off[i] = pool.size();
            for (auto& a : bus_alphas[i]) put_ext(pool, a);
            for (auto& b : betas[i]) put_ext(pool, b);
        }
        pool.push_back(0);
        DBuf pool_dev(&c, pool);
        GatherList gl;
        std::vector<DBuf> scratch;
        Section perm_section(&c);
        for (size_t i = 0; i < NC; i++) {
            uint32_t M = (uint32_t)machine_.airs[i].interactions.size();
            uint64_t n = main_nat[i]->height;
            perm_nat[i] = DMat(&c, n, 5 * (M + 1));
            vk::DMatView pv{nullptr, 0, 0, 0};
            if (prep_slot[i] >= 0) pv = prep_nat[prep_slot[i]].view();
            scratch.emplace_back(&c, (size_t)vk::perm_scratch_words(n));
            vk::launch_perm_trace(c.stream_for(i, n), main_nat[i]->view(), pv, iw_dev_[i].data, pool_dev.data + off[i], M, perm_nat[i].view(), scratch.back().data, fri_.interpret_air ? -2 : machine_.airs[i].native_chip);
            gl.add(perm_nat[i].data + (uint64_t)(5 * M) * n + (n - 1), n, 5, 0);
        }
        perm_section.join();
        c.check_launch("perm trace");
        DBuf gd(&c, gl.desc), gout(&c, gl.next_dst);
        vk::launch_gather(c.stream, gd.data, gl.n(), gout.data);
        if (gl.next_dst > CS_PINNED_WORDS) throw std::invalid_argument("prove: too many chips");
        cs_host = cs_pinned_;
        VG_HIP_CHECK(hipMemcpyAsync(cs_host, gout.data, gl.next_dst * 4, hipMemcpyDeviceToHost, c.stream));
        cs_keep = std::move(gout);
    }
    auto read_cumulative_sums = [&]() { for (size_t i = 0; i < NC; i++) cumulative_sums[i] = ext_from_canonical(cs_host + 5 * i); };
    if (dbg && dbg->check_constraints) { c.sync(); read_cumulative_sums(); }
    tm.perm = ms_since(t0);
    if (dbg && dbg->keep_matrices) {
        dbg->perm_traces.resize(NC);
        for (size_t i = 0; i < NC; i++) {
            auto& pm = perm_nat[i];
            DBuf tmp(&c, (size_t)(pm.height * pm.width));
            vk::launch_export_rows(c.stream, pm.view(), 0, pm.height, tmp.data);
            dbg->perm_traces[i].resize(pm.height * pm.width);
            c.download(dbg->perm_traces[i].data(), tmp.data, dbg->perm_traces[i].size() * 4);
        }
    }
    if (dbg && dbg->check_constraints) {
        std::vector<uint32_t> pool;
        std::vector<size_t> off(NC);
        std::vector<uint32_t> Ks(NC);
        for (size_t i = 0; i < NC; i++) {
            auto& air = machine_.airs[i];
            uint32_t M = (uint32_t)air.interactions.size(), K = air.program.num_asserts + M + 3;
            Ks[i] = K;
            off[i] = pool.size();
            Ext5 pw = Ext5::one();
// ... 597 lines not shown
```

### valida_amd/csrc/host/runtime.hpp

```cpp
#pragma once
#include <new>
#include <cstdio>
#include <cstdlib>
#include <hip/hip_runtime.h>
#include <cstring>
#include <atomic>
#include <map>
#include <mutex>
#include <stdexcept>
#include <string>
#include <tuple>
#include <vector>
#include "../kernels/launch.hpp"
#include "dense_lane.hpp"

namespace vhost {
using vg::Ext5;
using vg::Fp;

struct HipLaneApi {
    using Event = hipEvent_t;
    using Stream = hipStream_t;
    static Event create() { hipEvent_t e = nullptr; VG_HIP_CHECK(hipEventCreateWithFlags(&e, hipEventDisableTiming)); return e; }
    static void destroy(Event e) noexcept { if (e) (void)hipEventDestroy(e); }
    static bool record(Event e, Stream s) noexcept { return hipEventRecord(e, s) == hipSuccess; }
    static void wait(Stream s, Event e) { VG_HIP_CHECK(hipStreamWaitEvent(s, e, 0)); }
};
using HipDenseLane = DenseLane<HipLaneApi>;
inline HipDenseLane& dense_lane_of(int device) {
    static std::mutex* mu = new std::mutex;
    static std::map<int, HipDenseLane*>* lanes = new std::map<int, HipDenseLane*>;
    std::lock_guard<std::mutex> lk(*mu);
    HipDenseLane*& l = (*lanes)[device];
    if (!l) l = new HipDenseLane;
    return *l;
}

struct DeviceCtx {
    int device = 0;
    hipStream_t stream = nullptr;
    vk::DeviceTables tables{};
    std::multimap<size_t, void*> free_blocks;
    std::map<void*, size_t> live_blocks;
    size_t bytes_allocated = 0, peak_live = 0, live = 0;
    uint32_t* table_mem = nullptr;
    void* pinned = nullptr;
    size_t pinned_bytes = 0;
    uint8_t* stage = nullptr;
    static constexpr size_t STAGE_BYTES = 16u << 20;
    size_t stage_pos = 0;
    vk::Profiler profiler;
    int hash_kind = 0;
    const uint32_t* poseidon_tab = nullptr;
    bool poseidon_sparse = false;
    static constexpr int NUM_AUX = 1;
    hipStream_t aux[NUM_AUX] = {};
    hipEvent_t fork_ev = nullptr, join_ev[NUM_AUX] = {};
    hipEvent_t rider_ev = nullptr;
    uint32_t* rider_root_pin = nullptr;
    bool in_section = false;
    HipDenseLane* lane = nullptr;
    HipDenseLane::SlotPtr lane_slot;
    bool lane_on = true;
    uint64_t lane_min_nodes = 1ull << 18;
    std::atomic<uint64_t> lane_entered{0}, lane_waited{0};
    static const DeviceCtx*& lane_thread_ctx() { static thread_local const DeviceCtx* c = nullptr; return c; }
    bool lane_open_here() const { return lane_on && lane && lane_thread_ctx() == this; }
    std::vector<void*> deferred;
    std::mutex pool_mu;
    uint32_t poison_mode = 0, poison_word = 0;
    uint64_t poison_stats[4] = {0, 0, 0, 0};
    std::atomic<int> proofs_running{0};
    std::atomic<int> async_pending{0};
    std::mutex prove_mu;
    std::mutex upload_mu;
    hipStream_t upload_stream = nullptr;
    hipEvent_t upload_ev = nullptr;

    explicit DeviceCtx(int dev) : device(dev) {
        VG_HIP_CHECK(hipSetDevice(dev));
        VG_HIP_CHECK(hipStreamCreateWithFlags(&stream, hipStreamNonBlocking));
        for (int i = 0; i < NUM_AUX; i++) {
            VG_HIP_CHECK(hipStreamCreateWithFlags(&aux[i], hipStreamNonBlocking));
            VG_HIP_CHECK(hipEventCreateWithFlags(&join_ev[i], hipEventDisableTiming));
        }
        VG_HIP_CHECK(hipEventCreateWithFlags(&fork_ev, hipEventDisableTiming));
        VG_HIP_CHECK(hipEventCreateWithFlags(&rider_ev, hipEventDisableTiming));
        VG_HIP_CHECK(hipHostMalloc((void**)&rider_root_pin, 64));
        lane = &dense_lane_of(dev);
        lane_slot = std::make_shared<HipDenseLane::Slot>();
        init_tables();
    }
    void activate() {
        VG_HIP_CHECK(hipSetDevice(device));
        vk::g_profiler = &profiler;
    }
    ~DeviceCtx() {
        if (vk::g_profiler == &profiler) vk::g_profiler = nullptr;
        (void)hipSetDevice(device);
        (void)hipStreamSynchronize(stream);
        if (lane) lane->retire(lane_slot);
        for (int i = 0; i < NUM_AUX; i++) { (void)hipStreamSynchronize(aux[i]); (void)hipStreamDestroy(aux[i]); (void)hipEventDestroy(join_ev[i]); }
        (void)hipEventDestroy(fork_ev);
        if (rider_ev) (void)hipEventDestroy(rider_ev);
        if (rider_root_pin) (void)hipHostFree(rider_root_pin);
        if (sync_ev) (void)hipEventDestroy(sync_ev);
        for (auto& kv : free_blocks) (void)hipFree(kv.second);
        for (auto& kv : live_blocks) (void)hipFree(kv.first);
        if (table_mem) (void)hipFree(table_mem);
        for (auto& kv : lde_tabs) (void)hipFree(kv.second);
        if (upload_stream) { (void)hipStreamSynchronize(upload_stream); (void)hipStreamDestroy(upload_stream); (void)hipEventDestroy(upload_ev); }
        if (pinned) (void)hipHostFree(pinned);
        if (stage) (void)hipHostFree(stage);
        (void)hipStreamDestroy(stream);
    }
    DeviceCtx(const DeviceCtx&) = delete;

    void* alloc(size_t bytes) {
        std::lock_guard<std::mutex> lk(pool_mu);
        if (bytes == 0) bytes = 4;
        bytes = (bytes + 255) & ~(size_t)255;
        auto it = free_blocks.find(bytes);
        void* p;
        if (it != free_blocks.end()) { p = it->second; free_blocks.erase(it); }
        else {
            hipError_t e = hipMalloc(&p, bytes);
            if (e == hipErrorOutOfMemory) {
                (void)hipGetLastError();
                trim_locked();
                e = hipMalloc(&p, bytes);
            }
            if (e != hipSuccess) throw std::bad_alloc();
            bytes_allocated += bytes;
        }
        live_blocks[p] = bytes;
        live += bytes;
        if (live > peak_live) peak_live = live;
        if (poison_mode & 1) {
            if (!poison_fill_locked(p, bytes)) throw std::runtime_error("hip: the pool's poison fill failed");
            poison_stats[0]++; poison_stats[1] += bytes;
        }
        return p;
    }
    bool poison_fill_locked(void* p, size_t bytes) noexcept {
        int cur = -1;
        if (hipGetDevice(&cur) != hipSuccess) { (void)hipGetLastError(); cur = -1; }
        if (cur != device && hipSetDevice(device) != hipSuccess) { (void)hipGetLastError(); return false; }
        bool ok = hipDeviceSynchronize() == hipSuccess;
        ok = ok && hipMemsetD32((hipDeviceptr_t)p, (int)poison_word, bytes / 4) == hipSuccess;
        ok = ok && hipDeviceSynchronize() == hipSuccess;
// ... 217 lines not shown
```

### valida_amd/csrc/kernels/launch.hpp

```cpp
#pragma once
#include <vector>
#include "device_common.hpp"
#include "profiler.hpp"
#include "../air/symbolic.hpp"
#include "verify_args.hpp"

namespace vk {

struct QuotientArgs {
    DMatView main_lde, perm_lde, prep_lde;
    int log_n;
    const vair::Instr* prog;
    uint32_t n_instrs, n_regs, n_air_asserts;
    const uint32_t* iw;
    const uint32_t* consts;
    uint32_t K;
    uint32_t coset_shift, coset_shift_inv;
    int lqd;
    uint32_t zh_inv[8];
    uint32_t zh[8];
    uint32_t g_inv;
    DMatView out;
    int out_natural;
    static constexpr int INTERPRET = -2;
    int native_chip;
    const uint32_t* main_nx;
    const uint32_t* perm_nx;
    const uint32_t* prep_nx;
    uint32_t next_step_p1;
    QuotientArgs normalised() const {
        QuotientArgs b = *this;
        if (!b.main_nx) b.main_nx = b.main_lde.data;
        if (!b.perm_nx) b.perm_nx = b.perm_lde.data;
        if (!b.prep_nx) b.prep_nx = b.prep_lde.data;
        if (!b.next_step_p1) b.next_step_p1 = 1u + (1u << (b.lqd > 0 ? b.lqd : 1));
        return b;
    }
};

constexpr uint32_t INTERP_LDS_MIN_THREADS = 64;
constexpr uint32_t INTERP_LDS_BYTES_PAIR = 148 * 1024, INTERP_LDS_BYTES_GENERAL = 160 * 1024;
constexpr uint32_t INTERP_LDS_MAX_REGS_PAIR = INTERP_LDS_BYTES_PAIR / (4 * INTERP_LDS_MIN_THREADS);
constexpr uint32_t INTERP_LDS_MAX_REGS_GENERAL = INTERP_LDS_BYTES_GENERAL / (4 * INTERP_LDS_MIN_THREADS);
constexpr uint32_t interp_lds_max_regs(unsigned lqd) { return lqd == 1 ? INTERP_LDS_MAX_REGS_PAIR : INTERP_LDS_MAX_REGS_GENERAL; }
inline unsigned interp_lds_threads(uint32_t n_regs) {
    unsigned threads = 256;
    while (threads > INTERP_LDS_MIN_THREADS && (size_t)n_regs * threads * 4 > 64 * 1024) threads >>= 1;
    return threads;
}

void launch_ingest(hipStream_t st, const uint32_t* src_dev, DMatView dst, bool bitrev);
void launch_bitrev_rows(hipStream_t st, DMatView src, DMatView dst);
void launch_clock_probe(hipStream_t st, uint64_t* out3, uint32_t iters);
void launch_interleave_blocks(hipStream_t st, const uint32_t* src, uint32_t* dst, uint64_t rows, uint32_t log_wq, uint64_t n_cols);
void launch_export_rows(hipStream_t st, DMatView src, uint64_t row0, uint64_t nrows, uint32_t* dst_dev);
enum FieldProbeOp {
    FP_REDUCE_ONCE = 0, FP_SUB_MOD, FP_ADD, FP_SUB, FP_NEG, FP_MUL, FP_MONTY_REDUCE, FP_MONTY_REDUCE_WIDE, FP_FROM_CANONICAL, FP_CANONICAL, FP_INV,
    FP_EXT_MUL, FP_EXT_SQUARE, FP_EXT_SCALE, FP_EXT_INV, FP_BFLY_DIT_LB0, FP_BFLY_DIT, FP_BFLY_DIF_LB0, FP_BFLY_DIF, FP_MONTY_SIGNED, FP_SBOX, FP_SBOX_PLUS,
    FP_PERMUTE, FP_PERMUTE_PLAIN, FIELD_PROBE_OPS
};
bool field_probe_shape(uint32_t op, int* in_words, int* out_words);
void field_probe_check_twiddle_range(uint32_t op, const uint32_t* in_host, uint64_t n);
void launch_field_probe(hipStream_t st, uint32_t op, const uint32_t* in_dev, uint64_t n, const DeviceTables& tb, const uint32_t* pos_dev, bool sparse, uint32_t* out_dev);
void launch_intt(hipStream_t st, DMatView m, const DeviceTables& tb);
void launch_coset_ntt(hipStream_t st, DMatView coeffs, DMatView dst, uint64_t dst_row0, Fp shift, const DeviceTables& tb);
void launch_lde_natural(hipStream_t st, DMatView nat, DMatView lde, int log_blowup, const DeviceTables& tb, const LdeTables& lt, DMatView s1, DMatView s2);
void launch_verify_chunk(hipStream_t st, const VerifyChunkArgs& a);
void launch_keccak_leaves(hipStream_t st, const uint32_t* const* cols_dev, int n_elems, uint64_t n_rows, uint32_t* digests);
void launch_keccak_leaves_strided(hipStream_t st, const uint32_t* base, uint64_t stride, int n_elems, uint64_t n_rows, uint32_t* digests);
void launch_keccak_compress(hipStream_t st, const uint32_t* prev, const uint32_t* const* cols_dev, int n_elems, uint64_t n_out, uint32_t* next);
void launch_keccak_bottom_q(hipStream_t st, const uint32_t* jobs_dev, uint32_t n_jobs, const uint32_t* indices_dev, uint32_t* dst);
void launch_poseidon_bottom_q(hipStream_t st, const uint32_t* pos_dev, bool sparse, const uint32_t* jobs_dev, uint32_t n_jobs, const uint32_t* indices_dev, uint32_t* dst);
constexpr int KECCAK_TOP_MAX_LEVELS = 11;
struct KeccakTopArgs {
    const uint32_t* prev;
    uint64_t first_len;
    int levels;
    uint32_t* out[KECCAK_TOP_MAX_LEVELS];
    const uint32_t* const* cols[KECCAK_TOP_MAX_LEVELS];
    int n_elems[KECCAK_TOP_MAX_LEVELS];
    const uint32_t* leaf_base = nullptr;
    uint64_t leaf_stride = 0;
    int leaf_elems = 0;
    uint64_t leaf_rows = 0;
    uint64_t block_len = 0;
    const uint32_t* ch_pos = nullptr;
    uint32_t* ch_state = nullptr;
    uint32_t* ch_beta5 = nullptr;
    uint32_t* ch_commit8 = nullptr;
};
void launch_keccak_top(hipStream_t st, const KeccakTopArgs& a);
constexpr uint64_t KECCAK_LEVELS_BLOCK_LEN = 64;
void launch_keccak_levels(hipStream_t st, const KeccakTopArgs& a);
bool keccak_levels_fused(uint64_t len);
bool keccak_levels_take_leaves(uint64_t n_rows);
bool keccak_top_takes_leaves(uint64_t n_rows);
void launch_poseidon_leaves(hipStream_t st, const uint32_t* pos_dev, bool sparse, const uint32_t* const* cols_dev, int n_elems, uint64_t n_rows, uint32_t* digests);
void launch_poseidon_leaves_strided(hipStream_t st, const uint32_t* pos_dev, bool sparse, const uint32_t* base, uint64_t stride, int n_elems, uint64_t n_rows, uint32_t* digests);
void launch_poseidon_compress(hipStream_t st, const uint32_t* pos_dev, bool sparse, const uint32_t* prev, const uint32_t* const* cols_dev, int n_elems, uint64_t n_out, uint32_t* next);
bool poseidon_levels_take(uint64_t parents);
int poseidon_levels_group(uint64_t parents);
void launch_poseidon_levels(hipStream_t st, const uint32_t* pos_dev, bool sparse, const KeccakTopArgs& a);
void launch_poseidon_top(hipStream_t st, const uint32_t* pos_dev, bool sparse, const KeccakTopArgs& a);
uint64_t perm_scratch_words(uint64_t n);
void launch_add_ext_const(hipStream_t st, uint32_t* data, uint64_t stride, uint64_t n, const uint32_t* off5_dev);
void launch_perm_trace(hipStream_t st, DMatView main, DMatView prep, const uint32_t* iw_dev, const uint32_t* chal_dev, uint32_t M, DMatView perm,
                       uint32_t* scratch, int native_chip = -2);
void launch_quotient(hipStream_t st, const QuotientArgs& a, const DeviceTables& tb);
void launch_check_constraints(hipStream_t st, const QuotientArgs& a, unsigned long long* first_bad_dev);
struct TgCpuOp { uint32_t pc, fp, opcode; int32_t operands[5]; uint32_t kind, has_imm, imm, mem_first; };
struct TgMemOp { uint32_t clk, addr, value, is_write; };
struct TgAluOp { uint32_t opcode, a, b, c; };
struct TgOutOp { uint32_t clk, byte; };
enum { TG_CPU_STORE32 = 0, TG_CPU_LOAD32, TG_CPU_JAL, TG_CPU_JALV, TG_CPU_BEQ, TG_CPU_BNE, TG_CPU_IMM32, TG_CPU_BUS, TG_CPU_BUS_LEFT_IMM, TG_CPU_STOP,
       TG_CPU_LOADFP, TG_CPU_LOAD_U8, TG_CPU_LOAD_S8, TG_CPU_STORE_U8, TG_CPU_READ_ADVICE };
void launch_tracegen_cpu(hipStream_t st, const TgCpuOp* ops, uint64_t n, const TgMemOp* mem, uint64_t n_mem, DMatView t);
size_t tracegen_mem_sort_scratch_bytes(uint64_t n);
hipError_t launch_tracegen_mem(hipStream_t st, const TgMemOp* mem, uint64_t n, const uint32_t* static_cells, uint64_t n_static, uint32_t* keys2, uint32_t* idx2,
                               void* sort_tmp, size_t sort_tmp_bytes, DMatView t);
void launch_tracegen_alu(hipStream_t st, int chip, const TgAluOp* ops, uint64_t n, DMatView t);
void launch_tracegen_idle(hipStream_t st, int mode, const uint32_t* static_cells, uint64_t n_static, DMatView t);
hipError_t launch_tracegen_range(hipStream_t st, const TgCpuOp* ops, uint64_t n, const TgMemOp* mem, uint64_t n_mem, uint32_t* counts, DMatView t);
void launch_tracegen_alu2(hipStream_t st, int chip, const TgAluOp* ops, uint64_t n, DMatView t);
void launch_tracegen_output(hipStream_t st, const TgOutOp* vals, const uint32_t* row0, uint64_t n, uint64_t n_rows, DMatView t);
hipError_t launch_tracegen_program(hipStream_t st, const TgCpuOp* ops, uint64_t n, uint64_t padded_n, uint32_t rom_len, uint32_t* counts, DMatView t);
size_t bus_audit_sort_scratch_words(uint64_t n);
size_t bus_audit_scan_scratch_words(uint64_t n);
void launch_ba_records(hipStream_t st, const uint32_t* desc, uint32_t chip, uint64_t height, uint32_t width, uint32_t M, uint32_t hash_bits, unsigned long long* keys, uint32_t* ids,
                       uint32_t* cnt, uint32_t* live_out);
void launch_ba_iota(hipStream_t st, uint32_t* ids, uint64_t n);
void launch_ba_rekey(hipStream_t st, const uint32_t* desc, uint32_t chunk, const uint32_t* ids, const uint32_t* cnt, unsigned long long* keys, uint64_t n);
int launch_ba_sort(hipStream_t st, unsigned long long* keys2, uint32_t* vals2, uint64_t n, uint32_t* counts, const int* shifts, int n_shifts, int half);
void launch_ba_groups(hipStream_t st, const uint32_t* desc, const unsigned long long* keys, const uint32_t* ids, uint64_t n, bool exact, uint32_t* gid, uint32_t* head_pos,
                      uint32_t* scan_tmp, uint32_t* counters);
void launch_ba_reduce(hipStream_t st, const uint32_t* desc, const uint32_t* ids, const uint32_t* cnt, const uint32_t* gid, const uint32_t* head_pos, uint64_t n, bool check,
                      unsigned long long* sums, uint32_t* nrec, uint32_t* counters);
void launch_ba_select(hipStream_t st, const uint32_t* desc, const uint32_t* ids, const uint32_t* head_pos, const unsigned long long* sums, uint64_t n_groups_max, bool collect,
                      uint32_t cap, unsigned long long* ukeys, uint32_t* uvals, uint32_t* counters);
void launch_ba_report(hipStream_t st, const uint32_t* desc, const uint32_t* ids, const uint32_t* cnt, const uint32_t* head_pos, const unsigned long long* sums, const uint32_t* nrec,
                      const uint32_t* uvals, uint32_t n_rep, uint32_t R, uint32_t* out);
constexpr uint32_t CA_MAX_CONSTRAINTS = 96, CA_MASK_WORDS = 3;
constexpr int CA_INTERPRET = -2;
struct CaListed { uint32_t w[CA_MASK_WORDS]; };
struct CaArgs {
    const uint32_t* main;
    uint64_t mstride;
    const uint32_t* prep;
    uint64_t pstride;
    uint64_t n;
// ... 268 lines not shown
```

### valida_amd/csrc/kernels/layout.hip

```cpp
#include "launch.hpp"
#include <stdexcept>

namespace vk {

thread_local Profiler* g_profiler = nullptr;
thread_local ProfScope* g_scope = nullptr;

__global__ void k_ingest(const uint32_t* __restrict__ src, DMatView dst, int log_h, int bitrev) {
    extern __shared__ uint32_t lds[];
    const int W = (int)dst.width, LD = W | 1;
    const uint64_t j0 = (uint64_t)blockIdx.x * 64;
    const int rows = (int)((dst.height - j0) < 64 ? (dst.height - j0) : 64);
    const int lane = threadIdx.x & 63, wave = threadIdx.x >> 6, nwaves = blockDim.x >> 6;
    if (!bitrev) {
        const uint32_t* run = src + j0 * W;
        const int total = rows * W;
        int jr = (int)threadIdx.x / W, c = (int)threadIdx.x - jr * W;
        const int dj = (int)blockDim.x / W, dc = (int)blockDim.x - dj * W;
        int e = threadIdx.x;
        for (; e + 3 * (int)blockDim.x < total; e += 4 * blockDim.x) {
            uint32_t v[4];
#pragma unroll
            for (int u = 0; u < 4; u++) v[u] = run[e + u * (int)blockDim.x];
#pragma unroll
            for (int u = 0; u < 4; u++) {
                lds[jr * LD + c] = Fp::from_canonical(v[u]).v;
                jr += dj; c += dc;
                if (c >= W) { c -= W; jr++; }
            }
        }
        for (; e < total; e += blockDim.x) {
            lds[jr * LD + c] = Fp::from_canonical(run[e]).v;
            jr += dj; c += dc;
            if (c >= W) { c -= W; jr++; }
        }
    } else {
        for (int jr = wave; jr < rows; jr += nwaves) {
            uint64_t r = (uint64_t)vg::reverse_bits_len((uint32_t)(j0 + jr), (unsigned)log_h);
            const uint32_t* row = src + r * W;
            for (int c = lane; c < W; c += 64) lds[jr * LD + c] = Fp::from_canonical(row[c]).v;
        }
    }
    __syncthreads();
    for (int e = threadIdx.x; e < W * 64; e += blockDim.x) {
        int jr = e & 63, c = e >> 6;
        if (jr < rows) dst.data[(uint64_t)c * dst.stride + j0 + jr] = lds[jr * LD + c];
    }
}

__global__ void k_bitrev_rows(DMatView src, DMatView dst, int k) {
    __shared__ uint32_t tile[64][65];
    const uint32_t* s = src.col(blockIdx.y);
    uint32_t* d = dst.col(blockIdx.y);
    if (k < 12) {
        uint64_t n = 1ull << k;
        for (uint64_t r = (uint64_t)blockIdx.x * blockDim.x + threadIdx.x; r < n; r += (uint64_t)gridDim.x * blockDim.x)
            d[vg::reverse_bits_len((uint32_t)r, (unsigned)k)] = s[r];
        return;
    }
    const int midbits = k - 12;
    const uint32_t mid = blockIdx.x;
    for (int e = threadIdx.x; e < 4096; e += blockDim.x) {
        uint32_t lo = e & 63, hi = e >> 6;
        tile[hi][lo] = s[((uint64_t)hi << (k - 6)) | ((uint64_t)mid << 6) | lo];
    }
    __syncthreads();
    const uint32_t rmid = midbits ? vg::reverse_bits_len(mid, (unsigned)midbits) : 0;
    for (int e = threadIdx.x; e < 4096; e += blockDim.x) {
        uint32_t a = e & 63, b = e >> 6;
        uint32_t lo = vg::reverse_bits_len(b, 6), hi = vg::reverse_bits_len(a, 6);
        d[((uint64_t)b << (k - 6)) | ((uint64_t)rmid << 6) | a] = tile[hi][lo];
    }
}

__global__ void k_export_rows(DMatView src, uint64_t row0, uint64_t nrows, uint32_t* __restrict__ dst) {
    uint64_t total = nrows * src.width;
    for (uint64_t e = (uint64_t)blockIdx.x * blockDim.x + threadIdx.x; e < total; e += (uint64_t)gridDim.x * blockDim.x) {
        uint64_t r = e % nrows, c = e / nrows;
        dst[r * src.width + c] = src.get(row0 + r, c).canonical();
    }
}

__global__ void __launch_bounds__(256) k_interleave_blocks(const uint32_t* __restrict__ src, uint32_t* __restrict__ dst, uint64_t rows, uint32_t log_wq) {
    const uint64_t n = rows << log_wq, j = (uint64_t)blockIdx.x * blockDim.x + threadIdx.x;
    if (j >= n) return;
    const uint32_t eq = (uint32_t)(j & ((1u << log_wq) - 1u)), r = vg::reverse_bits_len(eq, log_wq);
    const uint64_t col = blockIdx.y;
    dst[col * n + j] = src[col * n + (uint64_t)r * rows + (j >> log_wq)];
}
void launch_interleave_blocks(hipStream_t st, const uint32_t* src, uint32_t* dst, uint64_t rows, uint32_t log_wq, uint64_t n_cols) {
    if (!log_wq) throw std::logic_error("interleave: one block is already in natural order");
    const uint64_t n = rows << log_wq;
    ProfScope ps("k_interleave_blocks", st, 8.0 * n * n_cols);
    VK_LAUNCH(k_interleave_blocks, dim3((unsigned)((n + 255) / 256), (unsigned)n_cols), dim3(256), 0, st, src, dst, rows, log_wq);
}

__global__ void k_clock_probe(uint64_t* out, uint32_t iters) {
    const uint64_t c0 = __builtin_readcyclecounter(), w0 = wall_clock64();
    uint32_t x = threadIdx.x;
    for (uint32_t i = 0; i < iters; i++) asm volatile("v_add_u32 %0, %0, %0" : "+v"(x));
    const uint64_t c1 = __builtin_readcyclecounter(), w1 = wall_clock64();
    if (threadIdx.x == 0) { out[0] = c1 - c0; out[1] = w1 - w0; out[2] = x; }
}
void launch_clock_probe(hipStream_t st, uint64_t* out3, uint32_t iters) { hipLaunchKernelGGL(k_clock_probe, dim3(1), dim3(64), 0, st, out3, iters); }

void launch_ingest(hipStream_t st, const uint32_t* src_dev, DMatView dst, bool bitrev) {
    int log_h = (int)vg::log2_strict_u64(dst.height);
    unsigned blocks = (unsigned)((dst.height + 63) / 64);
    size_t lds = (size_t)64 * (dst.width | 1) * 4;
    if (lds > 160 * 1024) throw std::invalid_argument("ingest: a matrix of " + std::to_string(dst.width) + " columns is wider than the 639 columns whose 64-row tile fits a workgroup's LDS");
    ProfScope ps("k_ingest", st, 8.0 * dst.height * dst.width);
    VK_LAUNCH(k_ingest, dim3(blocks), dim3(256), lds, st, src_dev, dst, log_h, bitrev ? 1 : 0);
}
void launch_bitrev_rows(hipStream_t st, DMatView src, DMatView dst) {
    int k = (int)vg::log2_strict_u64(src.height);
    ProfScope ps("k_bitrev_rows", st, 8.0 * src.height * src.width);
    unsigned bx = k < 12 ? (unsigned)(((1u << k) + 255) / 256) : (1u << (k - 12));
    VK_LAUNCH(k_bitrev_rows, dim3(bx, (unsigned)src.width), dim3(256), 0, st, src, dst, k);
}
void launch_export_rows(hipStream_t st, DMatView src, uint64_t row0, uint64_t nrows, uint32_t* dst_dev) {
    uint64_t total = nrows * src.width;
    unsigned blocks = (unsigned)((total + 255) / 256);
    if (blocks > 65535u * 16) blocks = 65535u * 16;
    if (blocks == 0) blocks = 1;
    ProfScope ps("k_export_rows", st, 8.0 * total);
    VK_LAUNCH(k_export_rows, dim3(blocks), dim3(256), 0, st, src, row0, nrows, dst_dev);
}

}
```

### valida_amd/csrc/kernels/ntt.hip

```cpp
#include "launch.hpp"
#include "butterfly.hpp"

namespace vk {

template <bool PAD> __device__ __forceinline__ int tile_addr(int i, int c, int LD) { return PAD ? i + (i >> 4) : i * LD + c; }

template <int R>
__device__ __forceinline__ void load_round_twiddles(Fp (&held)[(1 << R) - 1], const uint32_t* tw, int low, int lowbits) {
#pragma unroll
    for (int st = 0; st < R; st++) {
        const uint32_t* t = tw + ((1 << (lowbits + st)) - 1) + low;
#pragma unroll
        for (int k = 0; k < (1 << st); k++) held[(1 << st) - 1 + k] = Fp::raw(t[k << lowbits]);
    }
}

template <int R, bool DIT, bool PAD, int LB>
__device__ __forceinline__ void ntt_round(uint32_t* buf, const uint32_t* tw, int logn, int s_lo, int logT, int LD) {
    constexpr int G = 1 << R;
    const int n_items = (1 << (logn - R)) << logT;
    const int maskT = (1 << logT) - 1, lowbits = LB >= 0 ? LB : s_lo - 1, lowmask = (1 << lowbits) - 1;
    const bool linear = !PAD || lowbits >= 4 || lowbits + R <= 4;
    const int gs = PAD ? (lowbits >= 4 ? (1 << lowbits) + (1 << (lowbits - 4)) : (1 << lowbits)) : (LD << lowbits);
    for (int w = threadIdx.x; w < n_items; w += blockDim.x) {
// ... 257 lines not shown
            Fp cur = cur0;
            for (int i = threadIdx.x; i < n_lo; i += blockDim.x) { lds[tile_addr<true>(i, 0, 0)] = (Fp::raw(in[i]) * cur).v; cur *= step; }
        } else {
            commit_tile(pre, lds, n_lo);
        }
        __syncthreads();
        if (!from_src && t + gridDim.x < total) prefetch_tile(pre, tile_ptr(t + gridDim.x), n_lo);
        tile_transform<false, true>(lds, tw, k_lo, 0, 0);
        for (int i = threadIdx.x; i < n_lo; i += blockDim.x) out[i] = lds[tile_addr<true>(i, 0, 0)];
        __syncthreads();
    }
}


#ifndef VGPU_STRIDED_IO
#define VGPU_STRIDED_IO 1
#endif
#if defined(__HIP_DEVICE_COMPILE__)
#define VGPU_OPAQUE_S(x) asm volatile("" : "+s"(x))
#else
#define VGPU_OPAQUE_S(x) ((void)0)
#endif
__host__ __device__ constexpr uint32_t brev_c(uint32_t x, int bits) { uint32_t r = 0; for (int i = 0; i < bits; i++) r |= ((x >> i) & 1u) << (bits - 1 - i); return r; }
template <int K_HI, int LOGT> struct StridedShape {
    static constexpr int NT = 512, T = 1 << LOGT, LD = T + 1, NH = 1 << K_HI, LH = 9 - LOGT , HSTEP = 1 << LH, U = NH >> LH;
    static_assert(U == 32 && (K_HI - LH) == 5, "512 threads x 32 elements");
};
template <int K_HI, int LOGT, bool SRC_BITREV>
__device__ __forceinline__ void strided_tile_load(const uint32_t* col0, uint32_t n_lo, uint32_t* lds) {
    using S = StridedShape<K_HI, LOGT>;
    const uint32_t tid = threadIdx.x, c = tid & (S::T - 1), h0 = tid >> LOGT;
    const uint32_t blk0 = SRC_BITREV ? (__brev(h0) >> (32 - S::LH)) << 5 : h0;
    const uint32_t voff = (blk0 * n_lo + c) * 4u;
    uint32_t* l0 = lds + h0 * S::LD + c;
    const uint32_t step = (uint32_t)S::HSTEP * n_lo * 4u;
    uint32_t run = 0;
#pragma unroll
    for (int u0 = 0; u0 < S::U; u0 += 8) {
        uint32_t v[8];
#pragma unroll
        for (int k = 0; k < 8; k++) {
            const uint32_t u = (uint32_t)(u0 + k);
            if (SRC_BITREV) v[k] = load_at(col0, voff, brev_c(u, 5) * n_lo * 4u);
            else { v[k] = load_at(col0, voff, run); run += step; VGPU_OPAQUE_S(run); }
        }
#pragma unroll
        for (int k = 0; k < 8; k++) l0[(u0 + k) * S::HSTEP * S::LD] = v[k];
    }
}
template <int K_HI, int LOGT>
__device__ __forceinline__ void strided_tile_store(uint32_t* col0, uint32_t n_lo, const uint32_t* lds) {
    using S = StridedShape<K_HI, LOGT>;
    const uint32_t tid = threadIdx.x, c = tid & (S::T - 1), h0 = tid >> LOGT;
    const uint32_t voff = (h0 * n_lo + c) * 4u;
    const uint32_t* l0 = lds + h0 * S::LD + c;
    const uint32_t step = (uint32_t)S::HSTEP * n_lo * 4u;
    uint32_t run = 0;
#pragma unroll
    for (int u = 0; u < S::U; u++) { store_at(col0, voff, run, l0[u * S::HSTEP * S::LD]); run += step; VGPU_OPAQUE_S(run); }
}
template <int K_HI, int LOGT>
__device__ __forceinline__ void strided_tile_store_transposed(uint32_t* out_col, uint32_t tile, int k_lo, const uint32_t* lds) {
    using S = StridedShape<K_HI, LOGT>;
    const uint32_t tid = threadIdx.x, kq = (uint32_t)(k_lo - LOGT);
    const uint32_t qb_tile = kq ? __brev(tile) >> (32 - kq) : 0u;
    if (K_HI == 8) {
        const uint32_t p2 = tid & 255u, c0 = tid >> 8;
        uint32_t* base = out_col + ((uint64_t)qb_tile << K_HI);
        const uint32_t voff = ((((c0 << 5) << kq) << K_HI) + p2) * 4u;
        const uint32_t* l0 = lds + p2 * S::LD + c0;
#pragma unroll
        for (int i = 0; i < 32; i++) store_at(base, voff, ((brev_c((uint32_t)i, 5) << kq) << K_HI) * 4u, l0[2 * i]);
    } else {
        uint32_t* base = out_col + ((uint64_t)qb_tile << K_HI);
        const uint32_t* l0 = lds + tid * S::LD;
#pragma unroll
        for (int i = 0; i < 32; i++) {
            const uint32_t c = (uint32_t)(i >> 1), half = (uint32_t)(i & 1);
            store_at(base, (tid + 512u * half) * 4u, ((brev_c(c, LOGT) << kq) << K_HI) * 4u, l0[512 * half * S::LD + c]);
        }
    }
}

template <int FK_HI, int FLOGT>
__global__ void __launch_bounds__(FK_HI ? 512 : 1024) k_lde_a(DMatView src, DMatView dst, int k, int k_lo, int logT_arg, DeviceTables tb) {
    extern __shared__ uint32_t lds[];
    const int k_hi = FK_HI ? FK_HI : k - k_lo, logT = FK_HI ? FLOGT : logT_arg, n_hi = 1 << k_hi, T = 1 << logT, LD = T + 1;
    const uint64_t n_lo = 1ull << k_lo, r0 = (uint64_t)strided_tile_of_block(blockIdx.x, gridDim.x) * T;
    uint32_t* tw = lds + n_hi * LD;
    const uint32_t* in = src.col(blockIdx.y) + r0;
    uint32_t* out = dst.col(blockIdx.y) + r0;
    const int total = n_hi << logT;
    if constexpr (FK_HI != 0) strided_tile_load<FK_HI, FLOGT, false>(in, (uint32_t)n_lo, lds);
    else {
        int e = threadIdx.x;
        for (; e + 7 * (int)blockDim.x < total; e += 8 * blockDim.x) {
            uint32_t v[8];
#pragma unroll
            for (int u = 0; u < 8; u++) { const int eu = e + u * (int)blockDim.x; v[u] = in[(uint64_t)(eu >> logT) * n_lo + (eu & (T - 1))]; }
#pragma unroll
            for (int u = 0; u < 8; u++) { const int eu = e + u * (int)blockDim.x; lds[(eu >> logT) * LD + (eu & (T - 1))] = v[u]; }
        }
        for (; e < total; e += blockDim.x) { int c = e & (T - 1), h = e >> logT; lds[h * LD + c] = in[(uint64_t)h * n_lo + c]; }
    }
    stage_twiddles(tw, tb.itwc, k_hi);
    __syncthreads();
    if constexpr (FK_HI != 0) strided_transform<false, FK_HI, FLOGT>(lds, tw);
    else tile_transform<false, false>(lds, tw, k_hi, logT, LD);
    for (int p = threadIdx.x; p < n_hi; p += blockDim.x) {
        const uint32_t ca = __brev((uint32_t)p) >> (32 - k_hi);
        const Fp base = inv_root_pow(tb, k, ca);
        Fp cur = inv_root_pow(tb, k, (uint32_t)(((uint64_t)ca * r0) & ((1ull << k) - 1)));
        for (int c = 0; c < T; c++) { lds[p * LD + c] = (Fp::raw(lds[p * LD + c]) * cur).v; cur *= base; }
    }
    __syncthreads();
    if constexpr (FK_HI != 0) strided_tile_store<FK_HI, FLOGT>(out, (uint32_t)n_lo, lds);
    else
        for (int e = threadIdx.x; e < total; e += blockDim.x) { int c = e & (T - 1), h = e >> logT; out[(uint64_t)h * n_lo + c] = lds[h * LD + c]; }
}

template <int MAXT>
__global__ void __launch_bounds__(MAXT) k_lde_mid(DMatView src, DMatView dst, int k, int k_lo, int lb, DeviceTables tb, LdeTables lt) {
    extern __shared__ uint32_t lds[];
    const int n_lo = 1 << k_lo, k_hi = k - k_lo, n_hi = 1 << k_hi, b = 1 << lb;
    uint32_t* A = lds;
    uint32_t* W = lds + padded_words(n_lo);
    const uint64_t N = 1ull << k, tiles_per_col = (uint64_t)n_hi, total = tiles_per_col * src.width;
    const uint32_t nmask = (uint32_t)(N - 1);
    auto tile_ptr = [&](uint64_t t) { const uint64_t cidx = t >> k_hi; return src.col(cidx) + (t & (tiles_per_col - 1)) * n_lo; };
    uint32_t pre[CONTIG_MAX_PER_THREAD];
    if (blockIdx.x < total) prefetch_tile(pre, tile_ptr(blockIdx.x), n_lo);
    for (uint64_t t = blockIdx.x; t < total; t += gridDim.x) {
        const uint64_t cidx = t >> k_hi, p = t & (tiles_per_col - 1);
        commit_tile(pre, A, n_lo);
        __syncthreads();
        if (t + gridDim.x < total) prefetch_tile(pre, tile_ptr(t + gridDim.x), n_lo);
        tile_transform<false, true>(A, tb.itwc, k_lo, 0, 0);
        const uint32_t ca = k_hi ? __brev((uint32_t)p) >> (32 - k_hi) : 0u;
        for (int tc = 0; tc < b; tc++) {
            const uint32_t* fac = lt.fac + (size_t)tc * n_lo;
            for (int i = threadIdx.x; i < n_lo; i += blockDim.x) W[tile_addr<true>(i, 0, 0)] = (Fp::raw(A[tile_addr<true>(i, 0, 0)]) * Fp::raw(fac[i])).v;
            __syncthreads();
            tile_transform<true, true>(W, tb.twc, k_lo, 0, 0);
            if (k_hi > 0) {
                uint32_t* out = dst.col(cidx) + (uint64_t)tc * N + p * n_lo;
                const Fp step = root_pow(tb, k, (ca * blockDim.x) & nmask);
                Fp cur = Fp::raw(lt.sig[(size_t)tc * n_hi + ca]) * root_pow(tb, k, (ca * threadIdx.x) & nmask);
                for (int q = threadIdx.x; q < n_lo; q += blockDim.x) { out[q] = (Fp::raw(W[tile_addr<true>(q, 0, 0)]) * cur).v; cur *= step; }
            } else {
                const uint32_t blk = lb ? __brev((uint32_t)tc) >> (32 - lb) : 0u;
                uint32_t* out = dst.col(cidx) + (uint64_t)blk * N;
                for (int j = threadIdx.x; j < n_lo; j += blockDim.x) {
                    const int q = k ? (int)(__brev((uint32_t)j) >> (32 - k)) : 0;
                    out[j] = W[tile_addr<true>(q, 0, 0)];
                }
            }
            __syncthreads();
        }
    }
}

__global__ void __launch_bounds__(256) k_lde_mid12(DMatView src, DMatView dst, int k, int lb, DeviceTables tb, LdeTables lt) {
    extern __shared__ uint32_t lds[];
    constexpr int K_LO = 12, N_LO = 1 << K_LO;
    const int k_hi = k - K_LO, n_hi = 1 << k_hi, b = 1 << lb, tid = threadIdx.x;
    const uint64_t N = 1ull << k, tiles_per_col = (uint64_t)n_hi, total = tiles_per_col * src.width;
    const uint32_t nmask = (uint32_t)(N - 1);
    auto tile_ptr = [&](uint64_t t) { const uint64_t cidx = t >> k_hi; return src.col(cidx) + (t & (tiles_per_col - 1)) * N_LO; };
    Fp tw_in[15], tw_out[15];
    load_round_twiddles<4>(tw_in, tb.itwc, tid, 8);
    load_round_twiddles<4>(tw_out, tb.twc, tid, 8);
    const Fp* const held_in = tw_in;
    const Fp* const held_out = tw_out;
    uint32_t pre[16];
    if (blockIdx.x < total) {
        const uint32_t* sp = tile_ptr(blockIdx.x);
#pragma unroll
        for (int g = 0; g < 16; g++) pre[g] = sp[tid + 256 * g];
    }
    for (uint64_t t = blockIdx.x; t < total; t += gridDim.x) {
        const uint64_t cidx = t >> k_hi, p = t & (tiles_per_col - 1);
        Fp x[16];
#pragma unroll
        for (int g = 0; g < 16; g++) x[g] = Fp::raw(pre[g]);
        if (t + gridDim.x < total) {
            const uint32_t* sp = tile_ptr(t + gridDim.x);
#pragma unroll
            for (int g = 0; g < 16; g++) pre[g] = sp[tid + 256 * g];
        }
        butterflies<4, false, false>(x, tb.itwc, tid, 8, held_in);
        {
            uint32_t* p0 = lds + tile_addr<true>(tid, 0, 0);
#pragma unroll
            for (int g = 0; g < 16; g++) p0[g * 272] = x[g].v;
        }
        __syncthreads();
        ntt_round<4, false, true, 4>(lds, tb.itwc, 12, 5, 0, 0);
        {
            const uint32_t* p0 = lds + 17 * tid;
#pragma unroll
            for (int g = 0; g < 16; g++) x[g] = Fp::raw(p0[g]);
        }
        butterflies<4, false, true>(x, tb.itwc, 0, 0);
        const uint32_t ca = __brev((uint32_t)p) >> (32 - k_hi);
        const Fp step = root_pow(tb, k, (ca * 256u) & nmask), tw0 = root_pow(tb, k, (ca * (uint32_t)tid) & nmask);
        for (int tc = 0; tc < b; tc++) {
            Fp y[16];
            {
                const uint32_t* fac = lt.fac + (size_t)tc * N_LO + 16 * tid;
#pragma unroll
                for (int g = 0; g < 16; g++) y[g] = x[g] * Fp::raw(fac[g]);
            }
            butterflies<4, true, true>(y, tb.twc, 0, 0);
            {
                uint32_t* p0 = lds + 17 * tid;
#pragma unroll
                for (int g = 0; g < 16; g++) p0[g] = y[g].v;
            }
            __syncthreads();
            ntt_round<4, true, true, 4>(lds, tb.twc, 12, 5, 0, 0);
            {
                const uint32_t* p0 = lds + tile_addr<true>(tid, 0, 0);
#pragma unroll
                for (int g = 0; g < 16; g++) y[g] = Fp::raw(p0[g * 272]);
            }
            butterflies<4, true, false>(y, tb.twc, tid, 8, held_out);
            uint32_t* out = dst.col(cidx) + (uint64_t)tc * N + p * N_LO + tid;
            Fp cur = Fp::raw(lt.sig[(size_t)tc * n_hi + ca]) * tw0;
#pragma unroll
            for (int g = 0; g < 16; g++) { out[256 * g] = (y[g] * cur).v; cur *= step; }
            __syncthreads();
        }
    }
}

__global__ void __launch_bounds__(1024) k_lde_mid14(DMatView src, DMatView dst, int k, int lb, DeviceTables tb, LdeTables lt) {
    extern __shared__ uint32_t lds[];
    constexpr int K_LO = 14, N_LO = 1 << K_LO, NT = 1024;
    uint32_t* const coef = lds + (N_LO + (N_LO >> 4));
    const int k_hi = k - K_LO, n_hi = 1 << k_hi, b = 1 << lb, tid = threadIdx.x;
    const uint64_t N = 1ull << k, tiles_per_col = (uint64_t)n_hi, total = tiles_per_col * src.width;
    const uint32_t nmask = (uint32_t)(N - 1);
    for (uint64_t t = blockIdx.x; t < total; t += gridDim.x) {
        const uint64_t cidx = t >> k_hi, p = t & (tiles_per_col - 1);
        const uint32_t* sp = src.col(cidx) + p * N_LO;
#pragma unroll
        for (int j = 0; j < 4; j++) {
            const int w = tid + NT * j;
            Fp x4[4];
#pragma unroll
            for (int g = 0; g < 4; g++) x4[g] = Fp::raw(sp[w + 4096 * g]);
            butterflies<2, false, false>(x4, tb.itwc, w, 12);
#pragma unroll
            for (int g = 0; g < 4; g++) lds[tile_addr<true>(w + 4096 * g, 0, 0)] = x4[g].v;
        }
        __syncthreads();
        ntt_round<4, false, true, 8>(lds, tb.itwc, 14, 9, 0, 0);
        ntt_round<4, false, true, 4>(lds, tb.itwc, 14, 5, 0, 0);
        {
            Fp x[16];
            const uint32_t* p0 = lds + 17 * tid;
#pragma unroll
            for (int g = 0; g < 16; g++) x[g] = Fp::raw(p0[g]);
            butterflies<4, false, true>(x, tb.itwc, 0, 0);
            uint32_t* c0 = coef + 17 * tid;
#pragma unroll
            for (int g = 0; g < 16; g++) c0[g] = x[g].v;
        }
        const uint32_t ca = k_hi ? __brev((uint32_t)p) >> (32 - k_hi) : 0u;
        const Fp step = root_pow(tb, k, (ca * 4096u) & nmask);
        for (int tc = 0; tc < b; tc++) {
            Fp y[16];
            {
                const uint32_t* fac = lt.fac + (size_t)tc * N_LO + 16 * tid;
                const uint32_t* c0 = coef + 17 * tid;
#pragma unroll
                for (int g = 0; g < 16; g++) y[g] = Fp::raw(c0[g]) * Fp::raw(fac[g]);
            }
            butterflies<4, true, true>(y, tb.twc, 0, 0);
            {
                uint32_t* p0 = lds + 17 * tid;
#pragma unroll
                for (int g = 0; g < 16; g++) p0[g] = y[g].v;
            }
            __syncthreads();
            ntt_round<4, true, true, 4>(lds, tb.twc, 14, 5, 0, 0);
            ntt_round<4, true, true, 8>(lds, tb.twc, 14, 9, 0, 0);
            uint32_t* out = dst.col(cidx) + (uint64_t)tc * N + p * N_LO;
            const Fp sg = Fp::raw(lt.sig[(size_t)tc * n_hi + ca]);
#pragma unroll 1
            for (int j = 0; j < 4; j++) {
                const int w = tid + NT * j;
                Fp y4[4];
#pragma unroll
                for (int g = 0; g < 4; g++) y4[g] = Fp::raw(lds[tile_addr<true>(w + 4096 * g, 0, 0)]);
                butterflies<2, true, false>(y4, tb.twc, w, 12);
                Fp cur = sg * root_pow(tb, k, (ca * (uint32_t)w) & nmask);
#pragma unroll
                for (int g = 0; g < 4; g++) { out[w + 4096 * g] = (y4[g] * cur).v; cur *= step; }
            }
            __syncthreads();
        }
    }
}

template <int FK_HI, int FLOGT>
__global__ void __launch_bounds__(FK_HI ? 512 : 1024) k_lde_c(DMatView src, DMatView dst, int k, int k_lo, int lb, int logT_arg, DeviceTables tb
                        ) {
    extern __shared__ uint32_t lds[];
    const int k_hi = FK_HI ? FK_HI : k - k_lo, logT = FK_HI ? FLOGT : logT_arg, n_hi = 1 << k_hi, T = 1 << logT, LD = T + 1;
    const uint64_t n_lo = 1ull << k_lo, N = 1ull << k, q0 = (uint64_t)strided_tile_of_block(blockIdx.x, gridDim.x) * T;
    const uint32_t tc = blockIdx.z, blk = lb ? __brev(tc) >> (32 - lb) : 0u;
    uint32_t* tw = lds + n_hi * LD;
    const uint32_t* in = src.col(blockIdx.y) + (uint64_t)tc * N + q0;
    uint32_t* out = dst.col(blockIdx.y) + (uint64_t)blk * N;
    const int total = n_hi << logT;
    if constexpr (FK_HI != 0) strided_tile_load<FK_HI, FLOGT, true>(in, (uint32_t)n_lo, lds);
    else {
        int e = threadIdx.x;
        for (; e + 7 * (int)blockDim.x < total; e += 8 * blockDim.x) {
            uint32_t v[8];
#pragma unroll
            for (int u = 0; u < 8; u++) {
                const int eu = e + u * (int)blockDim.x;
                const uint32_t h = (uint32_t)(eu >> logT), pb = __brev(h) >> (32 - k_hi);
                v[u] = in[(uint64_t)pb * n_lo + (eu & (T - 1))];
            }
#pragma unroll
            for (int u = 0; u < 8; u++) { const int eu = e + u * (int)blockDim.x; lds[(eu >> logT) * LD + (eu & (T - 1))] = v[u]; }
        }
        for (; e < total; e += blockDim.x) {
            const int c = e & (T - 1);
            const uint32_t h = (uint32_t)(e >> logT), pb = __brev(h) >> (32 - k_hi);
            lds[h * LD + c] = in[(uint64_t)pb * n_lo + c];
        }
    }
    stage_twiddles(tw, tb.twc, k_hi);
    __syncthreads();
    if constexpr (FK_HI != 0) strided_transform<false, FK_HI, FLOGT>(lds, tw);
    else tile_transform<false, false>(lds, tw, k_hi, logT, LD);
    const uint32_t tile = strided_tile_of_block(blockIdx.x, gridDim.x);
    if constexpr (FK_HI != 0) strided_tile_store_transposed<FK_HI, FLOGT>(out, tile, k_lo, lds);
    else
    for (int e = threadIdx.x; e < total; e += blockDim.x) {
        const int p2 = e & (n_hi - 1), c = e >> k_hi;
        const uint32_t qb = __brev((uint32_t)(q0 + c)) >> (32 - k_lo);
        out[(uint64_t)qb * n_hi + p2] = lds[p2 * LD + c];
    }
}

struct NttPlan { int k, k_lo, k_hi, logT; unsigned threads_contig, threads_strided; size_t lds_contig, lds_strided; };
static NttPlan make_plan(int k) {
    NttPlan p;
    p.k = k; p.k_lo = k < 12 ? k : (k >= 23 ? 14 : 12); p.k_hi = k - p.k_lo;
    int t = 16384 >> p.k_hi; if (t > 64) t = 64; if (t < 8) t = 8;
    if ((1 << p.k_lo) < t) t = 1 << p.k_lo;
    p.logT = 0; while ((1 << p.logT) < t) p.logT++;
    unsigned n_lo = 1u << p.k_lo;
    p.threads_contig = n_lo / 16 < 64 ? 64 : (n_lo / 16 > 1024 ? 1024 : n_lo / 16);
    unsigned tile = (1u << p.k_hi) << p.logT;
    p.threads_strided = tile / 32 < 64 ? 64 : (tile / 32 > 1024 ? 1024 : tile / 32);
    if (p.threads_strided < (1u << p.logT)) p.threads_strided = 1u << p.logT;
    p.lds_contig = (size_t)padded_words((int)n_lo) * 4;
    p.lds_strided = ((size_t)(1u << p.k_hi) * ((1u << p.logT) + 1) + (1u << p.k_hi)) * 4;
    return p;
}

static void set_lds_limit() {
    static bool done = false;
    if (done) return;
    const int lim = 160 * 1024;
    (void)hipFuncSetAttribute((const void*)k_intt_strided, hipFuncAttributeMaxDynamicSharedMemorySize, lim);
    (void)hipFuncSetAttribute((const void*)k_ntt_strided, hipFuncAttributeMaxDynamicSharedMemorySize, lim);
    (void)hipFuncSetAttribute((const void*)k_intt_contig, hipFuncAttributeMaxDynamicSharedMemorySize, lim);
    (void)hipFuncSetAttribute((const void*)k_ntt_contig, hipFuncAttributeMaxDynamicSharedMemorySize, lim);
    (void)hipFuncSetAttribute((const void*)k_lde_a<0, 0>, hipFuncAttributeMaxDynamicSharedMemorySize, lim);
    (void)hipFuncSetAttribute((const void*)k_lde_a<8, 6>, hipFuncAttributeMaxDynamicSharedMemorySize, lim);
    (void)hipFuncSetAttribute((const void*)k_lde_a<10, 4>, hipFuncAttributeMaxDynamicSharedMemorySize, lim);
    (void)hipFuncSetAttribute((const void*)k_lde_mid<256>, hipFuncAttributeMaxDynamicSharedMemorySize, lim);
    (void)hipFuncSetAttribute((const void*)k_lde_mid<1024>, hipFuncAttributeMaxDynamicSharedMemorySize, lim);
    (void)hipFuncSetAttribute((const void*)k_lde_c<0, 0>, hipFuncAttributeMaxDynamicSharedMemorySize, lim);
    (void)hipFuncSetAttribute((const void*)k_lde_c<8, 6>, hipFuncAttributeMaxDynamicSharedMemorySize, lim);
    (void)hipFuncSetAttribute((const void*)k_lde_c<10, 4>, hipFuncAttributeMaxDynamicSharedMemorySize, lim);
    (void)hipFuncSetAttribute((const void*)k_lde_mid12, hipFuncAttributeMaxDynamicSharedMemorySize, lim);
    (void)hipFuncSetAttribute((const void*)k_lde_mid14, hipFuncAttributeMaxDynamicSharedMemorySize, lim);
    done = true;
}

void launch_intt(hipStream_t st, DMatView m, const DeviceTables& tb) {
    set_lds_limit();
    int k = (int)vg::log2_strict_u64(m.height);
    NttPlan p = make_plan(k);
    uint32_t ninv = Fp::from_canonical((uint32_t)(m.height % vg::P)).inv().v;
    const uint64_t tiles_c = (m.height >> p.k_lo) * m.width;
    dim3 gc((unsigned)(tiles_c < 4096 ? tiles_c : 4096));
    const double pass_bytes = 8.0 * m.height * m.width;
    {
        ProfScope ps("k_intt_contig", st, pass_bytes);
        VK_LAUNCH(k_intt_contig, gc, dim3(p.threads_contig), p.lds_contig, st, m, k, p.k_lo, tb, ninv);
    }
    if (p.k_hi > 0) {
        dim3 gs((unsigned)((1u << p.k_lo) >> p.logT), (unsigned)m.width);
        ProfScope ps("k_intt_strided", st, pass_bytes);
        VK_LAUNCH(k_intt_strided, gs, dim3(p.threads_strided), p.lds_strided, st, m, k, p.k_lo, p.logT, tb, ninv);
    }
}

void launch_coset_ntt(hipStream_t st, DMatView coeffs, DMatView dst, uint64_t dst_row0, Fp shift, const DeviceTables& tb) {
    set_lds_limit();
    int k = (int)vg::log2_strict_u64(coeffs.height);
    NttPlan p = make_plan(k);
    const uint64_t tiles_c = (coeffs.height >> p.k_lo) * coeffs.width;
    dim3 gc((unsigned)(tiles_c < 4096 ? tiles_c : 4096));
    const double pass_bytes = 8.0 * coeffs.height * coeffs.width;
    if (p.k_hi > 0) {
        dim3 gs((unsigned)((1u << p.k_lo) >> p.logT), (unsigned)coeffs.width);
        {
            CosetPowers cp;
            const unsigned hstep = p.threads_strided >> p.logT;
            Fp a = Fp::one(), s64 = shift.pow(64), sn = shift.pow(1ull << p.k_lo);
            for (int i = 0; i < 64; i++) { cp.lo[i] = a.v; a *= shift; }
            a = Fp::one();
            for (int i = 0; i < 256; i++) { cp.hi[i] = a.v; a *= s64; }
            a = Fp::one();
            cp.step = 0;
            for (unsigned i = 0; i < 128; i++) { cp.hp[i] = a.v; a *= sn; if (i + 1 == hstep) cp.step = a.v; }
            ProfScope ps("k_ntt_strided", st, pass_bytes);
            VK_LAUNCH(k_ntt_strided, gs, dim3(p.threads_strided), p.lds_strided, st, coeffs, dst, dst_row0, k, p.k_lo, p.logT, tb, cp);
        }
        ProfScope ps("k_ntt_contig", st, pass_bytes);
        VK_LAUNCH(k_ntt_contig, gc, dim3(p.threads_contig), p.lds_contig, st, coeffs, dst, dst_row0, k, p.k_lo, tb, shift.v, 0);
    } else {
        ProfScope ps("k_ntt_contig", st, pass_bytes);
        VK_LAUNCH(k_ntt_contig, gc, dim3(p.threads_contig), p.lds_contig, st, coeffs, dst, dst_row0, k, p.k_lo, tb, shift.v, 1);
    }
}

void launch_lde_natural(hipStream_t st, DMatView nat, DMatView lde, int log_blowup, const DeviceTables& tb, const LdeTables& lt, DMatView s1, DMatView s2) {
    set_lds_limit();
    const int k = (int)vg::log2_strict_u64(nat.height);
    NttPlan p = make_plan(k);
    const uint64_t tiles = ((uint64_t)1 << p.k_hi) * nat.width;
    dim3 gm((unsigned)(tiles < 4096 ? tiles : 4096));
    const size_t lds_mid = 2 * (size_t)padded_words(1 << p.k_lo) * 4;
    const double nw = 4.0 * nat.height * nat.width, b = (double)(1u << log_blowup);
    if (p.k_hi == 0) {
        ProfScope ps("k_lde_mid", st, nw * (1.0 + b));
        VK_LAUNCH(k_lde_mid<256>, gm, dim3(p.threads_contig), lds_mid, st, nat, lde, k, p.k_lo, log_blowup, tb, lt);
        return;
    }
    dim3 gs((unsigned)((1u << p.k_lo) >> p.logT), (unsigned)nat.width);
    {
        ProfScope ps("k_lde_a", st, 2.0 * nw);
        const int shape = VGPU_STRIDED_IO && VGPU_STRIDED_FIXED && p.threads_strided == 512 ? (p.k_hi == 8 && p.logT == 6 ? 8 : (p.k_hi == 10 && p.logT == 4 ? 10 : 0)) : 0;
        if (shape == 8) VK_LAUNCH((k_lde_a<8, 6>), gs, dim3(512), p.lds_strided, st, nat, s1, k, p.k_lo, p.logT, tb);
        else if (shape == 10) VK_LAUNCH((k_lde_a<10, 4>), gs, dim3(512), p.lds_strided, st, nat, s1, k, p.k_lo, p.logT, tb);
        else VK_LAUNCH((k_lde_a<0, 0>), gs, dim3(p.threads_strided), p.lds_strided, st, nat, s1, k, p.k_lo, p.logT, tb);
    }
    if (p.k_lo == 12) {
        if (gm.x > 4096u) gm.x = 4096u;
        ProfScope ps("k_lde_mid12", st, nw * (1.0 + b));
        VK_LAUNCH(k_lde_mid12, gm, dim3(256), (size_t)padded_words(4096) * 4, st, s1, s2, k, log_blowup, tb, lt);
    } else if (p.k_lo == 14) {
        ProfScope ps("k_lde_mid14", st, nw * (1.0 + b));
        VK_LAUNCH(k_lde_mid14, gm, dim3(1024), 2 * (size_t)padded_words(16384) * 4, st, s1, s2, k, log_blowup, tb, lt);
    } else {
        ProfScope ps("k_lde_mid", st, nw * (1.0 + b));
        if (p.threads_contig <= 256) VK_LAUNCH(k_lde_mid<256>, gm, dim3(p.threads_contig), lds_mid, st, s1, s2, k, p.k_lo, log_blowup, tb, lt);
        else VK_LAUNCH(k_lde_mid<1024>, gm, dim3(p.threads_contig), lds_mid, st, s1, s2, k, p.k_lo, log_blowup, tb, lt);
    }
    dim3 gc((unsigned)((1u << p.k_lo) >> p.logT), (unsigned)nat.width, 1u << log_blowup);
    ProfScope ps("k_lde_c", st, 2.0 * nw * b);
    const int shape_c = VGPU_STRIDED_IO && VGPU_STRIDED_FIXED && p.threads_strided == 512 ? (p.k_hi == 8 && p.logT == 6 ? 8 : (p.k_hi == 10 && p.logT == 4 ? 10 : 0)) : 0;
#define VG_LDE_C(A, B, THREADS) VK_LAUNCH((k_lde_c<A, B>), gc, dim3(THREADS), p.lds_strided, st, s2, lde, k, p.k_lo, log_blowup, p.logT, tb)
    if (shape_c == 8) VG_LDE_C(8, 6, 512);
    else if (shape_c == 10) VG_LDE_C(10, 4, 512);
    else VG_LDE_C(0, 0, p.threads_strided);
#undef VG_LDE_C
}

}
```

Before: 68.04 proofs/s.

## Detect constant trace columns at ingest and skip their LDE NTT work

The ingest kernel now flags, per column, whether any row differs from the first row. A column map built from those flags lets the LDE kernels run the NTT passes only on varying columns, while constant columns are filled directly with their value, since the low-degree extension of a constant is that constant. The aim is to avoid NTT work on the many constant or zero columns across the 14 chips. The cost is extra LDS and ballot work during ingest, a colmap kernel, a fill kernel, and more template instantiations. It is enabled by default and can be turned off with VGPU_CONST_COLS=0.

```diff
diff --git a/bindings/rust/src/lib.rs b/bindings/rust/src/lib.rs
--- a/bindings/rust/src/lib.rs
+++ b/bindings/rust/src/lib.rs
@@ -345,6 +345,7 @@
     pub fn vgpu_prover_trim(p: *mut VgpuProver) -> u64;
     pub fn vgpu_prover_memory_reset_peak(p: *mut VgpuProver);
     pub fn vgpu_prover_set_dense_lane(p: *mut VgpuProver, on: u32, min_nodes: u64);
+    pub fn vgpu_prover_set_const_columns(p: *mut VgpuProver, on: u32);
     pub fn vgpu_prover_lane_stats(p: *const VgpuProver, entered: *mut u64, waited: *mut u64);
     pub fn vgpu_prover_set_profiling(p: *mut VgpuProver, on: u32);
     pub fn vgpu_prover_set_prep_cache(p: *mut VgpuProver, on: u32);
@@ -356,6 +357,7 @@
     pub fn vgpu_trace_upload(p: *mut VgpuProver, data: *const u32, height: u64, width: u64, out: *mut *mut VgpuTrace) -> i32;
     pub fn vgpu_trace_free(t: *mut VgpuTrace);
     pub fn vgpu_commit_batches(p: *mut VgpuProver, mats: *const *const VgpuTrace, n_mats: u32, coset_shifts: *const u32, root: *mut u32, out: *mut *mut VgpuPdata) -> i32;
+    pub fn vgpu_commit_batches_flagged(p: *mut VgpuProver, mats: *const *const VgpuTrace, n_mats: u32, root: *mut u32, out: *mut *mut VgpuPdata, varies_out: *mut u32) -> i32;
     pub fn vgpu_pdata_lde(p: *mut VgpuProver, pd: *const VgpuPdata, idx: u32, out: *mut u32, cap_words: u64) -> i32;
     pub fn vgpu_pdata_num_matrices(pd: *const VgpuPdata) -> u32;
     pub fn vgpu_pdata_lde_view(pd: *const VgpuPdata, idx: u32, out: *mut VgpuLdeView) -> i32;
diff --git a/include/vgpu.h b/include/vgpu.h
--- a/include/vgpu.h
+++ b/include/vgpu.h
@@ -92,6 +92,7 @@
 uint64_t vgpu_prover_trim(vgpu_prover_t* p);
 void vgpu_prover_memory_reset_peak(vgpu_prover_t* p);
 void vgpu_prover_set_dense_lane(vgpu_prover_t* p, uint32_t on, uint64_t min_nodes);
+void vgpu_prover_set_const_columns(vgpu_prover_t* p, uint32_t on);
 void vgpu_prover_lane_stats(const vgpu_prover_t* p, uint64_t* entered, uint64_t* waited);
 
 void vgpu_prover_set_profiling(vgpu_prover_t* p, uint32_t on);
@@ -108,6 +109,8 @@
 
 int32_t vgpu_commit_batches(vgpu_prover_t* p, const vgpu_trace_t* const* mats, uint32_t n_mats, const uint32_t* coset_shifts,
                             uint32_t root[8], vgpu_pdata_t** out);
+int32_t vgpu_commit_batches_flagged(vgpu_prover_t* p, const vgpu_trace_t* const* mats, uint32_t n_mats, uint32_t root[8], vgpu_pdata_t** out,
+                                    uint32_t* varies_out);
 int32_t vgpu_pdata_lde(vgpu_prover_t* p, const vgpu_pdata_t* pd, uint32_t idx, uint32_t* out, uint64_t cap_words);
 typedef struct vgpu_lde_view {
     const uint32_t* data;
diff --git a/valida_amd/__init__.py b/valida_amd/__init__.py
--- a/valida_amd/__init__.py
+++ b/valida_amd/__init__.py
@@ -2079,8 +2079,13 @@
         _check(lib().vgpu_prover_create(ctypes.byref(cfg), machine._h, ctypes.byref(self._h)))
         if lane_off or int(lane_min or 0) > 0:
             self.set_dense_lane(not lane_off, int(lane_min or 0))
+        if os.environ.get("VGPU_CONST_COLS", "1") == "0":
+            self.set_const_columns(False)
         if poison is not None:
             self.set_pool_poison(poison)
+
+    def set_const_columns(self, on):
+        lib().vgpu_prover_set_const_columns(self._h, ctypes.c_uint32(1 if on else 0))
 
     def set_dense_lane(self, on, min_nodes=0):
         lib().vgpu_prover_set_dense_lane(self._h, ctypes.c_uint32(1 if on else 0), ctypes.c_uint64(int(min_nodes)))
@@ -2116,6 +2121,14 @@
         h = ctypes.c_void_p()
         _check(lib().vgpu_commit_batches(self._h, arr, ctypes.c_uint32(len(traces)), sh, root.ctypes.data_as(c_u32p), ctypes.byref(h)))
         return ProverData(self, h, root, [t.shape for t in traces])
+
+    def commit_batches_flagged(self, traces):
+        arr = (ctypes.c_void_p * len(traces))(*[t._h for t in traces])
+        root = np.zeros(8, dtype=np.uint32)
+        varies = np.zeros(sum(t.shape[1] for t in traces), dtype=np.uint32)
+        h = ctypes.c_void_p()
+        _check(lib().vgpu_commit_batches_flagged(self._h, arr, ctypes.c_uint32(len(traces)), root.ctypes.data_as(c_u32p), ctypes.byref(h), varies.ctypes.data_as(c_u32p)))
+        return ProverData(self, h, root, [t.shape for t in traces]), np.split(varies, np.cumsum([t.shape[1] for t in traces])[:-1])
 
     def generate_permutation_trace(self, chip, main, challenges, preprocessed=None):
         info = self.machine.chip_info(chip)
diff --git a/valida_amd/csrc/capi.cpp b/valida_amd/csrc/capi.cpp
--- a/valida_amd/csrc/capi.cpp
+++ b/valida_amd/csrc/capi.cpp
@@ -337,6 +337,12 @@
     if (live) *live = c.live;
     if (peak) *peak = c.peak_live;
 }
+void vgpu_prover_set_const_columns(vgpu_prover_t* p, uint32_t on) {
+    if (!p) return;
+    DeviceCtx& c = p->p->ctx();
+    std::lock_guard<std::mutex> lk(c.prove_mu);
+    c.const_cols_on = on != 0;
+}
 void vgpu_prover_set_dense_lane(vgpu_prover_t* p, uint32_t on, uint64_t min_nodes) {
     if (!p) return;
     DeviceCtx& c = p->p->ctx();
@@ -539,6 +545,40 @@
         pd->owner = p->p;
         pd->pd = commit_batches(&c, in, coset_shifts ? &shifts : nullptr, p->p->fri());
         memcpy(root, pd->pd->tree.root, 32);
+        *out = pd.release();
+    })
+}
+int32_t vgpu_commit_batches_flagged(vgpu_prover_t* p, const vgpu_trace_t* const* mats, uint32_t n_mats, uint32_t root[8], vgpu_pdata_t** out, uint32_t* varies_out) {
+    VG_TRY({
+        if (!p || !mats || !n_mats || !root || !out) throw std::invalid_argument("null argument");
+        DeviceCtx& c = p->p->ctx();
+        c.activate();
+        size_t words = 0;
+        for (uint32_t i = 0; i < n_mats; i++) {
+            if (!mats[i] || mats[i]->owner != p->p) throw std::invalid_argument("null trace or trace of another prover");
+            const DeviceTrace& t = *mats[i]->t;
+            if (!t.nat.empty()) throw std::invalid_argument("commit_batches_flagged: uploaded (row-major) matrices only");
+            if (t.height == 0 || (t.height & (t.height - 1))) throw std::invalid_argument("matrix height must be a power of two");
+            words += t.width;
+        }
+        DBuf flags(&c, words);
+        VG_HIP_CHECK(hipMemsetAsync(flags.data, 0, words * 4, c.stream));
+        std::vector<DMat> nat;
+        std::vector<CommitInput> in;
+        size_t off = 0;
+        for (uint32_t i = 0; i < n_mats; i++) {
+            const DeviceTrace& t = *mats[i]->t;
+            nat.emplace_back(&c, t.height, t.width);
+            vk::launch_ingest(c.stream, t.raw.data, nat.back().view(), false, flags.data + off);
+            off += t.width;
+        }
+        off = 0;
+        for (uint32_t i = 0; i < n_mats; i++) { in.push_back({&nat[i], false, false, c.const_cols_on ? flags.data + off : nullptr}); off += nat[i].width; }
+        std::unique_ptr<vgpu_pdata> pd(new vgpu_pdata());
+        pd->owner = p->p;
+        pd->pd = commit_batches(&c, in, nullptr, p->p->fri());
+        memcpy(root, pd->pd->tree.root, 32);
+        if (varies_out) c.download(varies_out, flags.data, words * 4);
         *out = pd.release();
     })
 }
diff --git a/valida_amd/csrc/host/pcs.hpp b/valida_amd/csrc/host/pcs.hpp
--- a/valida_amd/csrc/host/pcs.hpp
+++ b/valida_amd/csrc/host/pcs.hpp
@@ -190,6 +190,7 @@
     DMat* mat;
     bool rows_bitrev;
     bool consume;
+    const uint32_t* varies = nullptr;
 };
 
 inline DMat coset_lde(DeviceCtx* c, hipStream_t st, const CommitInput& in, unsigned log_blowup, Fp lde_shift) {
@@ -204,8 +205,13 @@
         const vk::LdeTables lt = c->lde_tables((int)k, (int)log_blowup, lde_shift);
         DMat s1, s2;
         if (k > 12) { s1 = DMat(c, n, in.mat->width); s2 = DMat(c, n * b, in.mat->width); }
+        DBuf colmap;
+        if (in.varies && k > 12) {
+            colmap = DBuf(c, vk::lde_colmap_words(in.mat->width));
+            vk::launch_lde_colmap(st, in.varies, in.mat->width, colmap.data);
+        }
         vk::launch_lde_natural(st, in.mat->view(), lde.view(), (int)log_blowup, c->tables, lt, s1.empty() ? vk::DMatView{nullptr, 0, 0, 0} : s1.view(),
-                               s2.empty() ? vk::DMatView{nullptr, 0, 0, 0} : s2.view());
+                               s2.empty() ? vk::DMatView{nullptr, 0, 0, 0} : s2.view(), colmap.data);
         c->check_launch("coset_lde");
         return lde;
     }
diff --git a/valida_amd/csrc/host/prover.cpp b/valida_amd/csrc/host/prover.cpp
--- a/valida_amd/csrc/host/prover.cpp
+++ b/valida_amd/csrc/host/prover.cpp
@@ -311,6 +311,20 @@
     std::vector<unsigned> log_deg(NC);
     std::vector<DMat> main_own(NC);
     std::vector<const DMat*> main_nat(NC);
+    const size_t NO_FLAGS = (size_t)-1;
+    std::vector<size_t> main_flags(NC, NO_FLAGS), prep_flags(preprocessed.size(), NO_FLAGS);
+    size_t flag_words = 0;
+    auto wants_flags = [&](const DeviceTrace* t) { return c.const_cols_on && t->nat.empty() && t->height > (1ull << 12) && t->width <= vk::INGEST_FLAGS_MAX_WIDTH; };
+    for (size_t i = 0; i < NC; i++)
+        if (wants_flags(main[i])) { main_flags[i] = flag_words; flag_words += main[i]->width; }
+    for (size_t k = 0; k < preprocessed.size(); k++)
+        if (wants_flags(preprocessed[k].second)) { prep_flags[k] = flag_words; flag_words += preprocessed[k].second->width; }
+    DBuf flags;
+    if (flag_words) {
+        flags = DBuf(&c, flag_words);
+        VG_HIP_CHECK(hipMemsetAsync(flags.data, 0, flag_words * 4, c.stream));
+    }
+    auto flags_at = [&](size_t off) -> uint32_t* { return off == NO_FLAGS ? nullptr : flags.data + off; };
     Section ingest_section(&c);
     for (size_t i = 0; i < NC; i++) {
         if (main[i]->width != machine_.airs[i].width) throw std::invalid_argument("prove: trace width mismatch for chip " + machine_.airs[i].name);
@@ -320,7 +334,7 @@
         if (!main[i]->nat.empty()) { main_nat[i] = &main[i]->nat; continue; }
         main_own[i] = DMat(&c, h, main[i]->width);
         main_nat[i] = &main_own[i];
-        vk::launch_ingest(c.stream_for(i, h), main[i]->raw.data, main_own[i].view(), false);
+        vk::launch_ingest(c.stream_for(i, h), main[i]->raw.data, main_own[i].view(), false, flags_at(main_flags[i]));
     }
     std::vector<std::pair<int, uint64_t>> prep_key;
     for (auto& pr : preprocessed) prep_key.emplace_back(pr.first, pr.second->uid);
@@ -340,7 +354,7 @@
         if (!t->nat.empty())
             VG_HIP_CHECK(hipMemcpyAsync(prep_nat[k].data, t->nat.data, t->height * t->width * 4, hipMemcpyDeviceToDevice, c.stream_for(k, t->height)));
         else
-            vk::launch_ingest(c.stream_for(k, t->height), t->raw.data, prep_nat[k].view(), false);
+            vk::launch_ingest(c.stream_for(k, t->height), t->raw.data, prep_nat[k].view(), false, flags_at(prep_flags[k]));
     }
     ingest_section.join();
     c.check_launch("ingest");
@@ -351,11 +365,11 @@
     std::vector<CommitInput> prep_in;
     const bool ride = !prep_nat.empty() && !prep_hit;
     if (ride)
-        for (auto& m : prep_nat) prep_in.push_back({&m, false, false});
+        for (size_t k = 0; k < prep_nat.size(); k++) prep_in.push_back({&prep_nat[k], false, false, flags_at(prep_flags[k])});
     std::unique_ptr<ProverData> main_pd;
     {
         std::vector<CommitInput> in;
-        for (auto m : main_nat) in.push_back({const_cast<DMat*>(m), false, false});
+        for (size_t i = 0; i < NC; i++) in.push_back({const_cast<DMat*>(main_nat[i]), false, false, flags_at(main_flags[i])});
         const CommitRider rider{&prep_in, &prep_pd_cache_};
         main_pd = commit_batches(&c, in, nullptr, fri_, ride ? &rider : nullptr);
     }
diff --git a/valida_amd/csrc/host/runtime.hpp b/valida_amd/csrc/host/runtime.hpp
--- a/valida_amd/csrc/host/runtime.hpp
+++ b/valida_amd/csrc/host/runtime.hpp
@@ -66,6 +66,7 @@
     std::atomic<uint64_t> lane_entered{0}, lane_waited{0};
     static const DeviceCtx*& lane_thread_ctx() { static thread_local const DeviceCtx* c = nullptr; return c; }
     bool lane_open_here() const { return lane_on && lane && lane_thread_ctx() == this; }
+    bool const_cols_on = true;
     std::vector<void*> deferred;
     std::mutex pool_mu;
     uint32_t poison_mode = 0, poison_word = 0;
diff --git a/valida_amd/csrc/kernels/launch.hpp b/valida_amd/csrc/kernels/launch.hpp
--- a/valida_amd/csrc/kernels/launch.hpp
+++ b/valida_amd/csrc/kernels/launch.hpp
@@ -49,7 +49,8 @@
     return threads;
 }
 
-void launch_ingest(hipStream_t st, const uint32_t* src_dev, DMatView dst, bool bitrev);
+void launch_ingest(hipStream_t st, const uint32_t* src_dev, DMatView dst, bool bitrev, uint32_t* varies = nullptr);
+constexpr uint64_t INGEST_FLAGS_MAX_WIDTH = 512;
 void launch_bitrev_rows(hipStream_t st, DMatView src, DMatView dst);
 void launch_clock_probe(hipStream_t st, uint64_t* out3, uint32_t iters);
 void launch_interleave_blocks(hipStream_t st, const uint32_t* src, uint32_t* dst, uint64_t rows, uint32_t log_wq, uint64_t n_cols);
@@ -64,7 +65,11 @@
 void launch_field_probe(hipStream_t st, uint32_t op, const uint32_t* in_dev, uint64_t n, const DeviceTables& tb, const uint32_t* pos_dev, bool sparse, uint32_t* out_dev);
 void launch_intt(hipStream_t st, DMatView m, const DeviceTables& tb);
 void launch_coset_ntt(hipStream_t st, DMatView coeffs, DMatView dst, uint64_t dst_row0, Fp shift, const DeviceTables& tb);
-void launch_lde_natural(hipStream_t st, DMatView nat, DMatView lde, int log_blowup, const DeviceTables& tb, const LdeTables& lt, DMatView s1, DMatView s2);
+void launch_lde_natural(hipStream_t st, DMatView nat, DMatView lde, int log_blowup, const DeviceTables& tb, const LdeTables& lt, DMatView s1, DMatView s2,
+                        const uint32_t* colmap = nullptr);
+constexpr uint32_t COLMAP_LIVE_COUNT = 0, COLMAP_CONST_COUNT = 1, COLMAP_LIVE = 2;
+inline size_t lde_colmap_words(uint64_t width) { return 2 + 2 * (size_t)width; }
+void launch_lde_colmap(hipStream_t st, const uint32_t* varies, uint64_t width, uint32_t* colmap);
 void launch_verify_chunk(hipStream_t st, const VerifyChunkArgs& a);
 void launch_keccak_leaves(hipStream_t st, const uint32_t* const* cols_dev, int n_elems, uint64_t n_rows, uint32_t* digests);
 void launch_keccak_leaves_strided(hipStream_t st, const uint32_t* base, uint64_t stride, int n_elems, uint64_t n_rows, uint32_t* digests);
diff --git a/valida_amd/csrc/kernels/layout.hip b/valida_amd/csrc/kernels/layout.hip
--- a/valida_amd/csrc/kernels/layout.hip
+++ b/valida_amd/csrc/kernels/layout.hip
@@ -6,7 +6,14 @@
 thread_local Profiler* g_profiler = nullptr;
 thread_local ProfScope* g_scope = nullptr;
 
-__global__ void k_ingest(const uint32_t* __restrict__ src, DMatView dst, int log_h, int bitrev) {
+__device__ __forceinline__ bool wave_any_elected(bool pred) {
+#if defined(__HIP_DEVICE_COMPILE__)
+    return __builtin_amdgcn_ballot_w64(pred) != 0 && (threadIdx.x & 63) == 0;
+#else
+    return pred;
+#endif
+}
+__global__ void k_ingest(const uint32_t* __restrict__ src, DMatView dst, int log_h, int bitrev, uint32_t* varies) {
     extern __shared__ uint32_t lds[];
     const int W = (int)dst.width, LD = W | 1;
     const uint64_t j0 = (uint64_t)blockIdx.x * 64;
@@ -41,10 +48,22 @@
             for (int c = lane; c < W; c += 64) lds[jr * LD + c] = Fp::from_canonical(row[c]).v;
         }
     }
+    if (varies)
+        for (int c = threadIdx.x; c < W; c += blockDim.x) lds[64 * LD + c] = Fp::from_canonical(src[c]).v;
     __syncthreads();
+    if (!varies) {
+        for (int e = threadIdx.x; e < W * 64; e += blockDim.x) {
+            int jr = e & 63, c = e >> 6;
+            if (jr < rows) dst.data[(uint64_t)c * dst.stride + j0 + jr] = lds[jr * LD + c];
+        }
+        return;
+    }
     for (int e = threadIdx.x; e < W * 64; e += blockDim.x) {
         int jr = e & 63, c = e >> 6;
-        if (jr < rows) dst.data[(uint64_t)c * dst.stride + j0 + jr] = lds[jr * LD + c];
+        const uint32_t first = lds[64 * LD + c];
+        const uint32_t v = jr < rows ? lds[jr * LD + c] : first;
+        if (jr < rows) dst.data[(uint64_t)c * dst.stride + j0 + jr] = v;
+        if (wave_any_elected(v != first)) varies[c] = 1;
     }
 }
 
@@ -95,6 +114,7 @@
     VK_LAUNCH(k_interleave_blocks, dim3((unsigned)((n + 255) / 256), (unsigned)n_cols), dim3(256), 0, st, src, dst, rows, log_wq);
 }
 
+#ifdef __HIPCC__
 __global__ void k_clock_probe(uint64_t* out, uint32_t iters) {
     const uint64_t c0 = __builtin_readcyclecounter(), w0 = wall_clock64();
     uint32_t x = threadIdx.x;
@@ -103,14 +123,16 @@
     if (threadIdx.x == 0) { out[0] = c1 - c0; out[1] = w1 - w0; out[2] = x; }
 }
 void launch_clock_probe(hipStream_t st, uint64_t* out3, uint32_t iters) { hipLaunchKernelGGL(k_clock_probe, dim3(1), dim3(64), 0, st, out3, iters); }
+#endif
 
-void launch_ingest(hipStream_t st, const uint32_t* src_dev, DMatView dst, bool bitrev) {
+void launch_ingest(hipStream_t st, const uint32_t* src_dev, DMatView dst, bool bitrev, uint32_t* varies) {
     int log_h = (int)vg::log2_strict_u64(dst.height);
     unsigned blocks = (unsigned)((dst.height + 63) / 64);
-    size_t lds = (size_t)64 * (dst.width | 1) * 4;
+    if (varies && dst.width > INGEST_FLAGS_MAX_WIDTH) throw std::invalid_argument("ingest: column flags are for matrices of at most " + std::to_string(INGEST_FLAGS_MAX_WIDTH) + " columns");
+    size_t lds = (size_t)(varies ? 65 : 64) * (dst.width | 1) * 4;
     if (lds > 160 * 1024) throw std::invalid_argument("ingest: a matrix of " + std::to_string(dst.width) + " columns is wider than the 639 columns whose 64-row tile fits a workgroup's LDS");
     ProfScope ps("k_ingest", st, 8.0 * dst.height * dst.width);
-    VK_LAUNCH(k_ingest, dim3(blocks), dim3(256), lds, st, src_dev, dst, log_h, bitrev ? 1 : 0);
+    VK_LAUNCH(k_ingest, dim3(blocks), dim3(256), lds, st, src_dev, dst, log_h, bitrev ? 1 : 0, varies);
 }
 void launch_bitrev_rows(hipStream_t st, DMatView src, DMatView dst) {
     int k = (int)vg::log2_strict_u64(src.height);
diff --git a/valida_amd/csrc/kernels/ntt.hip b/valida_amd/csrc/kernels/ntt.hip
--- a/valida_amd/csrc/kernels/ntt.hip
+++ b/valida_amd/csrc/kernels/ntt.hip
@@ -363,13 +363,18 @@
     }
 }
 
-template <int FK_HI, int FLOGT>
-__global__ void __launch_bounds__(FK_HI ? 512 : 1024) k_lde_a(DMatView src, DMatView dst, int k, int k_lo, int logT_arg, DeviceTables tb) {
-    extern __shared__ uint32_t lds[];
+template <int FK_HI, int FLOGT, bool MAPPED = false>
+__global__ void __launch_bounds__(FK_HI ? 512 : 1024) k_lde_a(DMatView src, DMatView dst, int k, int k_lo, int logT_arg, DeviceTables tb, const uint32_t* colmap) {
+    extern __shared__ uint32_t lds[];
+    uint64_t src_col = blockIdx.y;
+    if constexpr (MAPPED) {
+        if (blockIdx.y >= colmap[COLMAP_LIVE_COUNT]) return;
+        src_col = colmap[COLMAP_LIVE + blockIdx.y];
+    }
     const int k_hi = FK_HI ? FK_HI : k - k_lo, logT = FK_HI ? FLOGT : logT_arg, n_hi = 1 << k_hi, T = 1 << logT, LD = T + 1;
     const uint64_t n_lo = 1ull << k_lo, r0 = (uint64_t)strided_tile_of_block(blockIdx.x, gridDim.x) * T;
     uint32_t* tw = lds + n_hi * LD;
-    const uint32_t* in = src.col(blockIdx.y) + r0;
+    const uint32_t* in = src.col(src_col) + r0;
     uint32_t* out = dst.col(blockIdx.y) + r0;
     const int total = n_hi << logT;
     if constexpr (FK_HI != 0) strided_tile_load<FK_HI, FLOGT, false>(in, (uint32_t)n_lo, lds);
@@ -400,13 +405,13 @@
         for (int e = threadIdx.x; e < total; e += blockDim.x) { int c = e & (T - 1), h = e >> logT; out[(uint64_t)h * n_lo + c] = lds[h * LD + c]; }
 }
 
-template <int MAXT>
-__global__ void __launch_bounds__(MAXT) k_lde_mid(DMatView src, DMatView dst, int k, int k_lo, int lb, DeviceTables tb, LdeTables lt) {
+template <int MAXT, bool MAPPED = false>
+__global__ void __launch_bounds__(MAXT) k_lde_mid(DMatView src, DMatView dst, int k, int k_lo, int lb, DeviceTables tb, LdeTables lt, const uint32_t* colmap) {
     extern __shared__ uint32_t lds[];
     const int n_lo = 1 << k_lo, k_hi = k - k_lo, n_hi = 1 << k_hi, b = 1 << lb;
     uint32_t* A = lds;
     uint32_t* W = lds + padded_words(n_lo);
-    const uint64_t N = 1ull << k, tiles_per_col = (uint64_t)n_hi, total = tiles_per_col * src.width;
+    const uint64_t N = 1ull << k, tiles_per_col = (uint64_t)n_hi, total = tiles_per_col * (MAPPED ? (uint64_t)colmap[COLMAP_LIVE_COUNT] : src.width);
     const uint32_t nmask = (uint32_t)(N - 1);
     auto tile_ptr = [&](uint64_t t) { const uint64_t cidx = t >> k_hi; return src.col(cidx) + (t & (tiles_per_col - 1)) * n_lo; };
     uint32_t pre[CONTIG_MAX_PER_THREAD];
@@ -441,11 +446,12 @@
     }
 }
 
-__global__ void __launch_bounds__(256) k_lde_mid12(DMatView src, DMatView dst, int k, int lb, DeviceTables tb, LdeTables lt) {
+template <bool MAPPED>
+__global__ void __launch_bounds__(256) k_lde_mid12(DMatView src, DMatView dst, int k, int lb, DeviceTables tb, LdeTables lt, const uint32_t* colmap) {
     extern __shared__ uint32_t lds[];
     constexpr int K_LO = 12, N_LO = 1 << K_LO;
     const int k_hi = k - K_LO, n_hi = 1 << k_hi, b = 1 << lb, tid = threadIdx.x;
-    const uint64_t N = 1ull << k, tiles_per_col = (uint64_t)n_hi, total = tiles_per_col * src.width;
+    const uint64_t N = 1ull << k, tiles_per_col = (uint64_t)n_hi, total = tiles_per_col * (MAPPED ? (uint64_t)colmap[COLMAP_LIVE_COUNT] : src.width);
     const uint32_t nmask = (uint32_t)(N - 1);
     auto tile_ptr = [&](uint64_t t) { const uint64_t cidx = t >> k_hi; return src.col(cidx) + (t & (tiles_per_col - 1)) * N_LO; };
     Fp tw_in[15], tw_out[15];
@@ -515,12 +521,13 @@
     }
 }
 
-__global__ void __launch_bounds__(1024) k_lde_mid14(DMatView src, DMatView dst, int k, int lb, DeviceTables tb, LdeTables lt) {
+template <bool MAPPED>
+__global__ void __launch_bounds__(1024) k_lde_mid14(DMatView src, DMatView dst, int k, int lb, DeviceTables tb, LdeTables lt, const uint32_t* colmap) {
     extern __shared__ uint32_t lds[];
     constexpr int K_LO = 14, N_LO = 1 << K_LO, NT = 1024;
     uint32_t* const coef = lds + (N_LO + (N_LO >> 4));
     const int k_hi = k - K_LO, n_hi = 1 << k_hi, b = 1 << lb, tid = threadIdx.x;
-    const uint64_t N = 1ull << k, tiles_per_col = (uint64_t)n_hi, total = tiles_per_col * src.width;
+    const uint64_t N = 1ull << k, tiles_per_col = (uint64_t)n_hi, total = tiles_per_col * (MAPPED ? (uint64_t)colmap[COLMAP_LIVE_COUNT] : src.width);
     const uint32_t nmask = (uint32_t)(N - 1);
     for (uint64_t t = blockIdx.x; t < total; t += gridDim.x) {
         const uint64_t cidx = t >> k_hi, p = t & (tiles_per_col - 1);
@@ -585,16 +592,20 @@
     }
 }
 
-template <int FK_HI, int FLOGT>
-__global__ void __launch_bounds__(FK_HI ? 512 : 1024) k_lde_c(DMatView src, DMatView dst, int k, int k_lo, int lb, int logT_arg, DeviceTables tb
-                        ) {
-    extern __shared__ uint32_t lds[];
+template <int FK_HI, int FLOGT, bool MAPPED = false>
+__global__ void __launch_bounds__(FK_HI ? 512 : 1024) k_lde_c(DMatView src, DMatView dst, int k, int k_lo, int lb, int logT_arg, DeviceTables tb, const uint32_t* colmap) {
+    extern __shared__ uint32_t lds[];
+    uint64_t dst_col = blockIdx.y;
+    if constexpr (MAPPED) {
+        if (blockIdx.y >= colmap[COLMAP_LIVE_COUNT]) return;
+        dst_col = colmap[COLMAP_LIVE + blockIdx.y];
+    }
     const int k_hi = FK_HI ? FK_HI : k - k_lo, logT = FK_HI ? FLOGT : logT_arg, n_hi = 1 << k_hi, T = 1 << logT, LD = T + 1;
     const uint64_t n_lo = 1ull << k_lo, N = 1ull << k, q0 = (uint64_t)strided_tile_of_block(blockIdx.x, gridDim.x) * T;
     const uint32_t tc = blockIdx.z, blk = lb ? __brev(tc) >> (32 - lb) : 0u;
     uint32_t* tw = lds + n_hi * LD;
     const uint32_t* in = src.col(blockIdx.y) + (uint64_t)tc * N + q0;
-    uint32_t* out = dst.col(blockIdx.y) + (uint64_t)blk * N;
+    uint32_t* out = dst.col(dst_col) + (uint64_t)blk * N;
     const int total = n_hi << logT;
     if constexpr (FK_HI != 0) strided_tile_load<FK_HI, FLOGT, true>(in, (uint32_t)n_lo, lds);
     else {
@@ -628,6 +639,27 @@
         const uint32_t qb = __brev((uint32_t)(q0 + c)) >> (32 - k_lo);
         out[(uint64_t)qb * n_hi + p2] = lds[p2 * LD + c];
     }
+}
+
+__global__ void __launch_bounds__(256) k_lde_colmap(const uint32_t* __restrict__ varies, uint32_t width, uint32_t* __restrict__ colmap) {
+    extern __shared__ uint32_t lds[];
+    for (uint32_t j = threadIdx.x; j < width; j += blockDim.x) lds[j] = varies[j] != 0 ? 1u : 0u;
+    __syncthreads();
+    for (uint32_t j = threadIdx.x; j < width; j += blockDim.x) {
+        uint32_t rank = 0;
+        for (uint32_t i = 0; i < j; i++) rank += lds[i];
+        if (lds[j]) colmap[COLMAP_LIVE + rank] = j;
+        else colmap[COLMAP_LIVE + width + (j - rank)] = j;
+        if (j + 1 == width) { colmap[COLMAP_LIVE_COUNT] = rank + lds[j]; colmap[COLMAP_CONST_COUNT] = width - (rank + lds[j]); }
+    }
+}
+__global__ void __launch_bounds__(256) k_lde_fill_const(DMatView nat, DMatView lde, const uint32_t* __restrict__ colmap) {
+    if (blockIdx.y >= colmap[COLMAP_CONST_COUNT]) return;
+    const uint32_t c = colmap[COLMAP_LIVE + nat.width + blockIdx.y];
+    const uint32_t v = nat.col(c)[0];
+    uint4* out = reinterpret_cast<uint4*>(lde.col(c));
+    const uint64_t quads = lde.height >> 2;
+    for (uint64_t q = (uint64_t)blockIdx.x * blockDim.x + threadIdx.x; q < quads; q += (uint64_t)gridDim.x * blockDim.x) out[q] = make_uint4(v, v, v, v);
 }
 
 struct NttPlan { int k, k_lo, k_hi, logT; unsigned threads_contig, threads_strided; size_t lds_contig, lds_strided; };
@@ -663,8 +695,18 @@
     (void)hipFuncSetAttribute((const void*)k_lde_c<0, 0>, hipFuncAttributeMaxDynamicSharedMemorySize, lim);
     (void)hipFuncSetAttribute((const void*)k_lde_c<8, 6>, hipFuncAttributeMaxDynamicSharedMemorySize, lim);
     (void)hipFuncSetAttribute((const void*)k_lde_c<10, 4>, hipFuncAttributeMaxDynamicSharedMemorySize, lim);
-    (void)hipFuncSetAttribute((const void*)k_lde_mid12, hipFuncAttributeMaxDynamicSharedMemorySize, lim);
-    (void)hipFuncSetAttribute((const void*)k_lde_mid14, hipFuncAttributeMaxDynamicSharedMemorySize, lim);
+    (void)hipFuncSetAttribute((const void*)k_lde_mid12<false>, hipFuncAttributeMaxDynamicSharedMemorySize, lim);
+    (void)hipFuncSetAttribute((const void*)k_lde_mid14<false>, hipFuncAttributeMaxDynamicSharedMemorySize, lim);
+    (void)hipFuncSetAttribute((const void*)k_lde_a<0, 0, true>, hipFuncAttributeMaxDynamicSharedMemorySize, lim);
+    (void)hipFuncSetAttribute((const void*)k_lde_a<8, 6, true>, hipFuncAttributeMaxDynamicSharedMemorySize, lim);
+    (void)hipFuncSetAttribute((const void*)k_lde_a<10, 4, true>, hipFuncAttributeMaxDynamicSharedMemorySize, lim);
+    (void)hipFuncSetAttribute((const void*)k_lde_mid<256, true>, hipFuncAttributeMaxDynamicSharedMemorySize, lim);
+    (void)hipFuncSetAttribute((const void*)k_lde_mid<1024, true>, hipFuncAttributeMaxDynamicSharedMemorySize, lim);
+    (void)hipFuncSetAttribute((const void*)k_lde_c<0, 0, true>, hipFuncAttributeMaxDynamicSharedMemorySize, lim);
+    (void)hipFuncSetAttribute((const void*)k_lde_c<8, 6, true>, hipFuncAttributeMaxDynamicSharedMemorySize, lim);
+    (void)hipFuncSetAttribute((const void*)k_lde_c<10, 4, true>, hipFuncAttributeMaxDynamicSharedMemorySize, lim);
+    (void)hipFuncSetAttribute((const void*)k_lde_mid12<true>, hipFuncAttributeMaxDynamicSharedMemorySize, lim);
+    (void)hipFuncSetAttribute((const void*)k_lde_mid14<true>, hipFuncAttributeMaxDynamicSharedMemorySize, lim);
     done = true;
 }
 
@@ -717,7 +759,14 @@
     }
 }
 
-void launch_lde_natural(hipStream_t st, DMatView nat, DMatView lde, int log_blowup, const DeviceTables& tb, const LdeTables& lt, DMatView s1, DMatView s2) {
+void launch_lde_colmap(hipStream_t st, const uint32_t* varies, uint64_t width, uint32_t* colmap) {
+    if (width == 0 || width > 16384) throw std::invalid_argument("lde colmap: width out of range");
+    ProfScope ps("k_lde_colmap", st, 4.0 * 3 * width);
+    VK_LAUNCH(k_lde_colmap, dim3(1), dim3(256), (size_t)width * 4, st, varies, (uint32_t)width, colmap);
+}
+
+void launch_lde_natural(hipStream_t st, DMatView nat, DMatView lde, int log_blowup, const DeviceTables& tb, const LdeTables& lt, DMatView s1, DMatView s2,
+                        const uint32_t* colmap) {
     set_lds_limit();
     const int k = (int)vg::log2_strict_u64(nat.height);
     NttPlan p = make_plan(k);
@@ -727,33 +776,56 @@
     const double nw = 4.0 * nat.height * nat.width, b = (double)(1u << log_blowup);
     if (p.k_hi == 0) {
         ProfScope ps("k_lde_mid", st, nw * (1.0 + b));
-        VK_LAUNCH(k_lde_mid<256>, gm, dim3(p.threads_contig), lds_mid, st, nat, lde, k, p.k_lo, log_blowup, tb, lt);
+        VK_LAUNCH(k_lde_mid<256>, gm, dim3(p.threads_contig), lds_mid, st, nat, lde, k, p.k_lo, log_blowup, tb, lt, nullptr);
         return;
+    }
+    if (colmap) {
+        const uint64_t quads = lde.height >> 2, per_block = 256 * 16;
+        ProfScope ps("k_lde_fill_const", st, 0.0);
+        VK_LAUNCH(k_lde_fill_const, dim3((unsigned)((quads + per_block - 1) / per_block), (unsigned)nat.width), dim3(256), 0, st, nat, lde, colmap);
     }
     dim3 gs((unsigned)((1u << p.k_lo) >> p.logT), (unsigned)nat.width);
     {
         ProfScope ps("k_lde_a", st, 2.0 * nw);
         const int shape = VGPU_STRIDED_IO && VGPU_STRIDED_FIXED && p.threads_strided == 512 ? (p.k_hi == 8 && p.logT == 6 ? 8 : (p.k_hi == 10 && p.logT == 4 ? 10 : 0)) : 0;
-        if (shape == 8) VK_LAUNCH((k_lde_a<8, 6>), gs, dim3(512), p.lds_strided, st, nat, s1, k, p.k_lo, p.logT, tb);
-        else if (shape == 10) VK_LAUNCH((k_lde_a<10, 4>), gs, dim3(512), p.lds_strided, st, nat, s1, k, p.k_lo, p.logT, tb);
-        else VK_LAUNCH((k_lde_a<0, 0>), gs, dim3(p.threads_strided), p.lds_strided, st, nat, s1, k, p.k_lo, p.logT, tb);
+#define VG_LDE_A(A, B, THREADS)                                                                                                       \
+    do {                                                                                                                              \
+        if (colmap) VK_LAUNCH((k_lde_a<A, B, true>), gs, dim3(THREADS), p.lds_strided, st, nat, s1, k, p.k_lo, p.logT, tb, colmap);      \
+        else VK_LAUNCH((k_lde_a<A, B, false>), gs, dim3(THREADS), p.lds_strided, st, nat, s1, k, p.k_lo, p.logT, tb, colmap);           \
+    } while (0)
+        if (shape == 8) VG_LDE_A(8, 6, 512);
+        else if (shape == 10) VG_LDE_A(10, 4, 512);
+        else VG_LDE_A(0, 0, p.threads_strided);
+#undef VG_LDE_A
     }
     if (p.k_lo == 12) {
         if (gm.x > 4096u) gm.x = 4096u;
         ProfScope ps("k_lde_mid12", st, nw * (1.0 + b));
-        VK_LAUNCH(k_lde_mid12, gm, dim3(256), (size_t)padded_words(4096) * 4, st, s1, s2, k, log_blowup, tb, lt);
+        if (colmap) VK_LAUNCH(k_lde_mid12<true>, gm, dim3(256), (size_t)padded_words(4096) * 4, st, s1, s2, k, log_blowup, tb, lt, colmap);
+        else VK_LAUNCH(k_lde_mid12<false>, gm, dim3(256), (size_t)padded_words(4096) * 4, st, s1, s2, k, log_blowup, tb, lt, colmap);
     } else if (p.k_lo == 14) {
         ProfScope ps("k_lde_mid14", st, nw * (1.0 + b));
-        VK_LAUNCH(k_lde_mid14, gm, dim3(1024), 2 * (size_t)padded_words(16384) * 4, st, s1, s2, k, log_blowup, tb, lt);
+        const size_t lds14 = 2 * (size_t)padded_words(16384) * 4;
+        if (colmap) VK_LAUNCH(k_lde_mid14<true>, gm, dim3(1024), lds14, st, s1, s2, k, log_blowup, tb, lt, colmap);
+        else VK_LAUNCH(k_lde_mid14<false>, gm, dim3(1024), lds14, st, s1, s2, k, log_blowup, tb, lt, colmap);
     } else {
         ProfScope ps("k_lde_mid", st, nw * (1.0 + b));
-        if (p.threads_contig <= 256) VK_LAUNCH(k_lde_mid<256>, gm, dim3(p.threads_contig), lds_mid, st, s1, s2, k, p.k_lo, log_blowup, tb, lt);
-        else VK_LAUNCH(k_lde_mid<1024>, gm, dim3(p.threads_contig), lds_mid, st, s1, s2, k, p.k_lo, log_blowup, tb, lt);
+        if (p.threads_contig <= 256) {
+            if (colmap) VK_LAUNCH((k_lde_mid<256, true>), gm, dim3(p.threads_contig), lds_mid, st, s1, s2, k, p.k_lo, log_blowup, tb, lt, colmap);
+            else VK_LAUNCH(k_lde_mid<256>, gm, dim3(p.threads_contig), lds_mid, st, s1, s2, k, p.k_lo, log_blowup, tb, lt, colmap);
+        } else {
+            if (colmap) VK_LAUNCH((k_lde_mid<1024, true>), gm, dim3(p.threads_contig), lds_mid, st, s1, s2, k, p.k_lo, log_blowup, tb, lt, colmap);
+            else VK_LAUNCH(k_lde_mid<1024>, gm, dim3(p.threads_contig), lds_mid, st, s1, s2, k, p.k_lo, log_blowup, tb, lt, colmap);
+        }
     }
     dim3 gc((unsigned)((1u << p.k_lo) >> p.logT), (unsigned)nat.width, 1u << log_blowup);
     ProfScope ps("k_lde_c", st, 2.0 * nw * b);
     const int shape_c = VGPU_STRIDED_IO && VGPU_STRIDED_FIXED && p.threads_strided == 512 ? (p.k_hi == 8 && p.logT == 6 ? 8 : (p.k_hi == 10 && p.logT == 4 ? 10 : 0)) : 0;
-#define VG_LDE_C(A, B, THREADS) VK_LAUNCH((k_lde_c<A, B>), gc, dim3(THREADS), p.lds_strided, st, s2, lde, k, p.k_lo, log_blowup, p.logT, tb)
+#define VG_LDE_C(A, B, THREADS)                                                                                                              \
+    do {                                                                                                                                     \
+        if (colmap) VK_LAUNCH((k_lde_c<A, B, true>), gc, dim3(THREADS), p.lds_strided, st, s2, lde, k, p.k_lo, log_blowup, p.logT, tb, colmap); \
+        else VK_LAUNCH((k_lde_c<A, B, false>), gc, dim3(THREADS), p.lds_strided, st, s2, lde, k, p.k_lo, log_blowup, p.logT, tb, colmap);     \
+    } while (0)
     if (shape_c == 8) VG_LDE_C(8, 6, 512);
     else if (shape_c == 10) VG_LDE_C(10, 4, 512);
     else VG_LDE_C(0, 0, p.threads_strided);
```

Result: faster. 69.40 proofs/s, median of 6 (+2.0%).
